# tdj28/ml-depth-pro-video

Hardware: AMD Instinct MI355X
Metric: frames/sec at 1536x1536 (1/2/4/8 MI355X) + depth L1 vs reference (higher is better)
Workload: dtype bf16+f16; 1 GPU; BASELINE config 2/3: one 1536x1536 frame per GPU per step through DepthPro.infer (patch+image+FOV ViT-L, decoder, heads), hipGraph replay; global_batch=1, parallelism=frame-dp1, graph=True

## Files before the change

ml-depth-pro-video_amd/csrc/dp_gemm.hip:

```cpp
#include "dp_gemm_impl.h"
#include "dp_ln_merge.h"

namespace dpg {
std::atomic<int> g_dbg_flags{0};

constexpr int DP_MAX_DEV = 64;
std::atomic<int> g_num_cu[DP_MAX_DEV];
int num_cus() {
  int dev = 0;
  if (hipGetDevice(&dev) != hipSuccess || dev < 0) dev = 0;
  std::atomic<int>& slot = g_num_cu[dev < DP_MAX_DEV ? dev : 0];
  int n = slot.load(std::memory_order_relaxed);
  if (n <= 0) {
    if (hipDeviceGetAttribute(&n, hipDeviceAttributeMultiprocessorCount, dev) != hipSuccess || n <= 0) n = 256;
    if (dev < DP_MAX_DEV) slot.store(n, std::memory_order_relaxed);
  }
  return n;
}
}

namespace {
int launch_tile(const GemmP& p, int tile, bool conv, bool bf16, void* ws, hipStream_t s) {
  switch (tile_info(tile).fam) {
    case FAM_SMALL: return launch_part_small(p, tile, conv, bf16, s);
    case FAM_BIG320: return launch_part_big320(p, tile, conv, bf16, s);
    case FAM_8PH: return launch_part_8ph(p, tile, conv, bf16, s);
    case FAM_8PH320: return launch_part_8ph320(p, conv, bf16, s);
    case FAM_PBIG: return launch_part_pbig(p, tile, conv, bf16, s);
    case FAM_SK: return launch_part_sk(p, conv, ws, bf16, s);
    case FAM_SPLITK: return launch_part_splitk(p, conv, bf16, s);
    case FAM_CV3: return launch_part_cv3(p, conv, bf16, s, tile_info(tile).bm / 16);
    default: return launch_part_big(p, tile, conv, bf16, s);
  }
}
}

extern "C" int dp_gemm_debug_flags(int flags) {
  g_dbg_flags.store(flags, std::memory_order_relaxed);
  return 0;
}

extern "C" int64_t dp_gemm_workspace_size(void) { return SK_FLAG_BYTES + (int64_t)SK_MAX_WG * SK_TILE_F * 4; }

namespace {
__global__ void __launch_bounds__(256) ln_merge_kernel(const float* __restrict__ part, int M, float eps,
                                                       float* __restrict__ out) {
  const int m = blockIdx.x * 256 + threadIdx.x;
  if (m >= M) return;
  const f32x4_t* pp = (const f32x4_t*)(part + (long long)m * 16);
  f32x4_t c[4];
  #pragma unroll
  for (int i = 0; i < 4; ++i) c[i] = pp[i];
  *(float2*)(out + 2LL * m) = ln_merge_row(c, eps);
}

__global__ void ws_check_kernel(uint32_t* __restrict__ ws, int32_t* __restrict__ status) {
  const uint32_t err = ws[DP_GEMM_WS_ERROR_OFFSET / 4];
  if (threadIdx.x == 0) status[0] = (int32_t)err;
  if (err == 0) return;
  __syncthreads();
  for (int i = threadIdx.x; i < (int)(SK_FLAG_BYTES / 4); i += blockDim.x) ws[i] = 0u;
}
}

extern "C" int dp_gemm_workspace_check(void* workspace, int32_t* status, dp_stream_t stream) {
  if (!workspace || !status) return DP_ERR_ARG;
  hipLaunchKernelGGL(ws_check_kernel, dim3(1), dim3(256), 0, (hipStream_t)stream, (uint32_t*)workspace, status);
  DP_CHECK_LAUNCH();
  return 0;
}

namespace {
struct PlanFacts {
  bool conv, k3s1p1, sq3x3, hps, hps4, bc, lnp, lnc, ws_ok, col8_shape, col8_align, off32, dcv;
  long long tiles256;
  unsigned c_bytes, dcv_bytes;
};

PlanFacts plan_facts(const dp_gemm_args* a) {
  PlanFacts f{};
  f.conv = a->a_mode == DP_A_CONV;
  f.k3s1p1 = f.conv && a->k_h == 3 && a->k_w == 3 && a->stride == 1 && a->pad == 1;
  f.sq3x3 = f.k3s1p1 && a->in_h == a->in_w && a->out_h == a->in_h && a->out_w == a->in_w && a->in_w % 16 == 0 &&
            a->in_c % 64 == 0 && (long long)a->M * a->in_c < (1LL << 30);
  f.hps = a->store_mode == DP_STORE_HEAD_PS;
  f.hps4 = f.k3s1p1 && f.hps && a->K == 4 * a->in_c;
  f.bc = a->store_mode == DP_STORE_ROWS && a->head_corr;
  f.lnp = a->ln_part_out || a->ln_xb_out || a->ln_xl || a->ln_rs_out;
  f.lnc = a->ln_part_in || a->ln_colsum || a->ln_rs_in;
  f.ws_ok = a->workspace && a->workspace_bytes >= dp_gemm_workspace_size();
  f.col8_shape = a->N % 8 == 0 && !(a->store_mode == DP_STORE_DECONV2X2 && a->dc_cout % 8 != 0);
  f.col8_align = !(a->c_dtype != DP_F32 && a->ldc % 8 != 0) && !(a->R1 && a->ldr1 % 8 != 0) &&
                 !(a->R2 && a->ldr2 % 8 != 0);
  f.tiles256 = (long long)((a->M + 255) / 256) * (a->N / 256);
  if (a->store_mode == DP_STORE_ROWS && !a->head_w && !a->head_corr) {
    long long last = a->M - 1;
    if (a->row_group) last = (last / a->row_group) * a->row_group_out + a->row_off + last % a->row_group;
    const long long ext = (last * a->ldc + a->N) * (a->c_dtype == DP_F32 ? 4 : 2);
    if (ext < 0xFFFFFF00LL) f.c_bytes = (unsigned)ext;
  }
  if (a->store_mode == DP_STORE_DECONV2X2 && a->c_dtype != DP_F32) {
    const long long ext = ((4LL * a->M - 1) * a->ldc + a->dc_cout) * 2;
    if (ext < 0xFFFFFF00LL) f.dcv_bytes = (unsigned)ext;
  }
  f.off32 = (a->a_mode != DP_A_DENSE || (long long)a->M * a->lda < (1LL << 31)) &&
            (long long)a->N * a->ldb < (1LL << 31);
  if (!f.off32) f.c_bytes = f.dcv_bytes = 0;
  f.dcv = a->store_mode == DP_STORE_DECONV2X2 && !a->relu_a && !a->gamma && a->act == DP_ACT_NONE &&
          a->dc_w >= 8;
  return f;
}

int validate(const dp_gemm_args* a, const PlanFacts& f) {
  if (a->M <= 0 || a->N <= 0 || a->K <= 0) return DP_ERR_SHAPE;
  if (a->K % BK != 0 || a->N % 4 != 0) return DP_ERR_SHAPE;
  if (a->ldb % 8 != 0 || (a->a_mode == DP_A_DENSE && a->lda % 8 != 0)) return DP_ERR_ALIGN;
  if ((!a->head_w && !f.hps && a->ldc % 4 != 0) || (a->R1 && a->ldr1 % 4 != 0) ||
      (a->R2 && a->ldr2 % 4 != 0) || (a->pos && a->ldpos % 4 != 0))
    return DP_ERR_ALIGN;
  if (!a->A || !a->B || (!a->C && !a->ln_xl)) return DP_ERR_ARG;
  if (a->dtype != DP_BF16 && a->dtype != DP_F16) return DP_ERR_DTYPE;
  if (a->c_dtype != DP_BF16 && a->c_dtype != DP_F16 && a->c_dtype != DP_F32) return DP_ERR_DTYPE;
  if (a->c_dtype != DP_F32 && a->c_dtype != a->dtype) return DP_ERR_DTYPE;
  if (a->accumulate && a->c_dtype != DP_F32) return DP_ERR_DTYPE;
  if (a->pos && (a->pos_group <= 0)) return DP_ERR_ARG;
  if (f.conv) {
    if (a->in_c % BK != 0 || (a->k_h * a->k_w * a->in_c != a->K && !f.hps4)) return DP_ERR_SHAPE;
    if (a->out_h <= 0 || a->out_w <= 0 || a->stride <= 0 || a->M % (a->out_h * a->out_w) != 0)
      return DP_ERR_SHAPE;
  }
  if (f.hps) {
    if (!f.conv || a->N != 128 || !a->head_w || !a->head_corr || a->c_dtype != DP_F32 ||
        a->accumulate || a->R1 || a->R2 || a->pos || a->gamma || a->act != DP_ACT_NONE)
      return DP_ERR_ARG;
  }
  if (f.bc) {
    if (!f.k3s1p1 || a->head_w || a->relu_a ||
        a->row_group || a->out_h != a->in_h || a->out_w != a->in_w || a->N % 8 != 0 || a->N < 128 ||
        (a->tile != DP_TILE_AUTO && a->tile <= DP_TILE_256x32))
      return DP_ERR_ARG;
  }
  if (a->store_mode == DP_STORE_DECONV2X2) {
    if (a->dc_cout % 4 != 0 || a->N != 4 * a->dc_cout || a->dc_h <= 0 || a->dc_w <= 0 ||
        a->M % (a->dc_h * a->dc_w) != 0)
      return DP_ERR_SHAPE;
  }
  if (f.lnp && f.lnc) return DP_ERR_ARG;
  if (f.lnp && !a->ln_xl && (!a->ln_part_out || !a->ln_xb_out || !a->accumulate || !a->C || a->c_dtype != DP_F32 ||
                             a->act != DP_ACT_NONE || a->N % 256 != 0))
    return DP_ERR_ARG;
  if (a->ln_xl && (!a->ln_xb_out || !a->accumulate || a->c_dtype != DP_F32 || a->act != DP_ACT_NONE ||
                   a->N % 256 != 0 || a->ldc % 8 != 0 || (long long)a->M * a->ldc * 4 >= 0xFFFFFF00LL))
    return DP_ERR_ARG;
  if (f.lnc && (!(a->ln_part_in || a->ln_rs_in) || (a->ln_part_in && a->ln_rs_in) || !a->ln_colsum || a->K != 1024 ||
                a->accumulate || a->c_dtype == DP_F32 || a->gamma || (a->act != DP_ACT_NONE && a->act != DP_ACT_GELU) ||
                !(a->ln_eps > 0.f)))
    return DP_ERR_ARG;
  if (a->ln_rs_out && (!a->ln_xl || !a->ln_part_out || a->N != 1024 || !(a->ln_eps > 0.f) || !f.ws_ok ||
                       (a->M + 319) / 320 > 1023 - LN_CNT_WORD))
    return DP_ERR_ARG;
  if (a->ln_rs_in && a->tile != DP_TILE_AUTO && a->tile != DP_TILE_P8PH_256x256) return DP_ERR_ARG;
  if ((f.lnp || f.lnc) && a->tile != DP_TILE_AUTO && a->tile != DP_TILE_8PH_320x256 &&
      !(f.lnc && a->tile == DP_TILE_P8PH_256x256))
    return DP_ERR_ARG;
  return 0;
}

int col8_rc(const PlanFacts& f, int tile) {
  if (tile < 0 || !tile_info(tile).col8) return 0;
  return !f.col8_shape ? DP_ERR_SHAPE : !f.col8_align ? DP_ERR_ALIGN : 0;
}
bool serves_streamk(const dp_gemm_args* a, const PlanFacts& f) { return f.ws_ok && a->N % 256 == 0; }
bool serves_splitk(const dp_gemm_args* a, const PlanFacts& f, int& split) {
  if (!f.ws_ok || a->N % 256 != 0 || a->store_mode != DP_STORE_ROWS || a->row_group || a->head_w || a->head_corr ||
      f.lnp || f.lnc) return false;
  const long long slab = (long long)a->M * a->N * 4, slabs = (a->workspace_bytes - SK_FLAG_BYTES) / slab;
  split = (int)std::min({num_cus() / f.tiles256, (long long)(a->K / BK / 2), slabs, 32LL});
  return true;
}

bool serves_pbig(const dp_gemm_args* a, const PlanFacts& f) { return f.c_bytes && a->N % 256 == 0; }

bool serves_p8ph(const dp_gemm_args* a, const PlanFacts& f, int dbg) {
  return a->a_mode == DP_A_DENSE && a->N % 256 == 0 && a->K >= 128 && a->c_dtype != DP_F32 &&
         ((a->store_mode == DP_STORE_ROWS && f.c_bytes) || (f.dcv && f.dcv_bytes)) && !a->R1 && !a->R2 && !a->pos &&
         !a->accumulate && !a->row_group && !a->head_w && !a->head_corr && !(dbg & DBG_NO_FAST_EPILOGUE);
}

bool serves_8ph320(const dp_gemm_args* a, const PlanFacts& f, int dbg) {
  const bool plain = a->a_mode == DP_A_DENSE && !a->relu_a && a->N % 256 == 0 && a->store_mode == DP_STORE_ROWS &&
                     !a->R1 && !a->R2 && !a->pos && !a->row_group && !a->head_w && !a->head_corr &&
                     !(dbg & DBG_NO_FAST_EPILOGUE) && f.off32;
  const bool epi_ok = (!a->accumulate && a->c_dtype != DP_F32) ||
                      (a->accumulate && a->c_dtype == DP_F32 && a->act == DP_ACT_NONE);
  return plain && epi_ok;
}

bool cv3_shape(const dp_gemm_args* a, const PlanFacts& f, int th) {
  if (!f.sq3x3 || a->out_w % th != 0 || a->row_group || (a->head_w && !f.hps) || a->gamma || a->pos || a->accumulate)
    return false;
  if (!f.hps && a->store_mode != DP_STORE_ROWS) return false;
  if (f.hps4 && a->relu_a) return false;
  if (f.bc && (a->c_dtype == DP_F32 || a->R1 || a->R2 || a->N % 128 != 0)) return false;
  if (!f.hps && !f.bc && (a->c_dtype == DP_F32 || a->N % 256 != 0)) return false;
  return th == 12 ? !(f.hps || f.bc) : th == 24 ? (f.hps || f.bc) && a->N == 128 : true;
}
bool serves_cv3(const dp_gemm_args* a, const PlanFacts& f, int th) {
  return cv3_shape(a, f, th) && (a->act == DP_ACT_NONE || a->act == DP_ACT_RELU) && (long long)a->N * a->ldb < (1LL << 31);
}

int choose_auto(const dp_gemm_args* a, const PlanFacts& f, int dbg) {
  auto ncu = [n = 0LL]() mutable { return n ? n : n = num_cus(); };
  const long long tiles256 = f.tiles256, tiles320 = (long long)((a->M + 319) / 320) * (a->N / 256);
  int tile;
  if (a->N <= 32) tile = DP_TILE_256x32;
  else if (a->N <= 64) tile = DP_TILE_256x64;
  else if (!f.col8_shape || !f.col8_align) tile = DP_TILE_128x128;
  else if (a->N == 128 && a->M >= 512 * 256) {
    tile = !f.bc || (dbg & DBG_NO_CV3_HEAD) ? DP_TILE_BIG_512x128 : cv3_shape(a, f, 24) ? DP_TILE_CV3_384x128
           : cv3_shape(a, f, 16) ? DP_TILE_CV3_256x256 : DP_TILE_BIG_512x128;
  }
  else if (a->N % 256 != 0) tile = DP_TILE_BIG_256x128;
  else if (serves_streamk(a, f) && f.conv && !(dbg & DBG_NO_SMALL_STREAMK) && tiles256 < ncu() && a->K >= 4608) {
    tile = DP_TILE_STREAMK_256x256;
  } else if (serves_streamk(a, f) && a->K <= 256 && tiles256 >= 1024) {
    tile = DP_TILE_STREAMK_256x256;
  } else {
    const long long tiles128 = (long long)((a->M + 255) / 256) * (a->N / 128);
    const long long cost256 = (tiles256 + ncu() - 1) / ncu() * 256 * 20, cost320 = (tiles320 + ncu() - 1) / ncu() * 320 * 20;
    const long long cost128 = (tiles128 + ncu() - 1) / ncu() * 128 * 23;
    if (cost128 < cost256 && cost128 < cost320) tile = DP_TILE_BIG_256x128;
    else if (cost320 < cost256) tile = DP_TILE_BIG_320x256;
    else tile = (tiles256 >= 600 && !f.conv) ? DP_TILE_8PH_256x256 : DP_TILE_BIG_256x256;
    if (tile == DP_TILE_8PH_256x256 && (dbg & DBG_FC1_BIG320)) tile = DP_TILE_BIG_320x256;
    else if (tile == DP_TILE_8PH_256x256 && (dbg & DBG_FC1_BIG256)) tile = DP_TILE_BIG_256x256;
  }
  if (serves_pbig(a, f) && !(dbg & DBG_NO_PBIG)) {
    const bool dense_ok = f.conv || (dbg & DBG_PBIG_DENSE);
    if (dense_ok && tile == DP_TILE_BIG_320x256 && tiles320 >= 2 * ncu()) tile = DP_TILE_PBIG_320x256;
    else if (dense_ok && tile == DP_TILE_BIG_256x256 && tiles256 >= 2 * ncu()) tile = DP_TILE_PBIG_256x256;
  }
  if (f.dcv && f.col8_shape && f.col8_align && !(dbg & DBG_NO_P8PH_DECONV) && tiles256 >= 128) tile = DP_TILE_P8PH_256x256;
  else if (tile == DP_TILE_8PH_256x256 && !(dbg & DBG_NO_P8PH) && serves_p8ph(a, f, dbg)) tile = DP_TILE_P8PH_256x256;
  if (tile == DP_TILE_BIG_320x256 && !(dbg & DBG_NO_8PH320) && serves_8ph320(a, f, dbg)) tile = DP_TILE_8PH_320x256;
  if (!(dbg & DBG_NO_CV3) && !f.bc && a->N % 256 == 0 && f.col8_align && cv3_shape(a, f, 16) && f.off32 &&
      a->act != DP_ACT_GELU) {
    const long long t16 = (long long)(a->M / 256) * (a->N / 256);
    if (t16 >= 4 * ncu()) tile = DP_TILE_CV3_256x256;
    else if (cv3_shape(a, f, 12)) {
      const long long t12 = (long long)(a->M / ((long long)a->in_w * a->in_w)) * (a->in_w / 12) * (a->in_w / 16) * (a->N / 256);
      if (t12 >= 2 * ncu() && t12 % ncu() == 0 && t16 % ncu() != 0) tile = DP_TILE_CV3_192x256;
      else if (t12 <= ncu() && 2 * t12 >= ncu()) tile = DP_TILE_CV3_192x256;
    }
  }
  return tile;
}

void fill_params(const dp_gemm_args* a, const PlanFacts& f, int tile, int ksplit, int dbg, GemmP& p) {
  p.M = a->M; p.N = a->N; p.K = a->K;
  p.A = (const u16*)a->A; p.lda = a->lda;
  p.B = (const u16*)a->B; p.ldb = a->ldb;
  p.relu_a = a->relu_a;
  p.in_h = a->in_h; p.in_w = a->in_w; p.in_c = a->in_c; p.k_h = a->k_h; p.k_w = a->k_w;
  p.stride = a->stride; p.pad = a->pad; p.out_h = a->out_h; p.out_w = a->out_w;
  p.bias = a->bias; p.act = a->act; p.gamma = a->gamma;
  p.pos = a->pos; p.ldpos = a->ldpos; p.pos_group = a->pos_group; p.pos_off = a->pos_off;
  p.R1 = (const u16*)a->R1; p.ldr1 = a->ldr1; p.R2 = (const u16*)a->R2; p.ldr2 = a->ldr2;
  p.C = a->C; p.ldc = a->ldc; p.c_dtype = a->c_dtype; p.accumulate = a->accumulate;
  p.store_mode = a->store_mode; p.dc_h = a->dc_h; p.dc_w = a->dc_w; p.dc_cout = a->dc_cout;
  p.row_group = a->row_group; p.row_group_out = a->row_group_out; p.row_off = a->row_off;
  p.head_w = a->head_w; p.head_b = a->head_b; p.head_corr = a->head_corr;
  p.ln_part_out = a->ln_part_out; p.ln_xb_out = (u16*)a->ln_xb_out; p.ln_xl = (u16*)a->ln_xl;
  p.ln_part_in = a->ln_part_in; p.ln_colsum = a->ln_colsum; p.ln_eps = a->ln_eps;
  p.ln_rs = a->ln_rs_in; p.ln_rs_out = a->ln_rs_out;
  p.ln_cnt = a->ln_rs_out ? (unsigned*)a->workspace + LN_CNT_WORD : nullptr;
  p.tiles_n = p.tiles_m = 1;
  if (tile == DP_TILE_STREAMK_256x256) p.tiles_n = a->N / 256, p.tiles_m = (a->M + 255) / 256;
  p.dbg = dbg;
  p.c_bytes = tile == DP_TILE_P8PH_256x256 && f.dcv ? f.dcv_bytes : f.c_bytes;
  p.ksplit = ksplit;
  p.kpart = ksplit > 1 ? (float*)((char*)a->workspace + SK_FLAG_BYTES) : nullptr;
  p.groups = 1;
}

int gemm_plan(const dp_gemm_args* a, GemmP& p, int& tile) {
  if (!a) return DP_ERR_ARG;
  const PlanFacts f = plan_facts(a);
  if (const int rc = validate(a, f)) return rc;
  const int dbg = g_dbg_flags.load(std::memory_order_relaxed);
  tile = a->tile;
  if (a->ln_rs_in) tile = DP_TILE_P8PH_256x256;
  if (f.hps) {
    if (f.hps4) {
      if (tile == DP_TILE_AUTO) tile = a->out_w % 48 == 0 ? DP_TILE_CV3_384x128 : DP_TILE_CV3_256x256;
      else if (tile != DP_TILE_CV3_256x256 && tile != DP_TILE_CV3_384x128) return DP_ERR_ARG;
    } else if (tile != DP_TILE_CV3_256x256 && tile != DP_TILE_CV3_384x128 && tile != DP_TILE_BIG_256x128)
      tile = a->M >= 512 * 256 ? DP_TILE_BIG_512x128 : DP_TILE_BIG_256x128;
  } else if (a->head_w) {
    if (a->N > 32 || a->store_mode != DP_STORE_ROWS) return DP_ERR_SHAPE;
    tile = DP_TILE_256x32;
  }
  if (const int rc = col8_rc(f, tile)) return rc;
  if (tile == DP_TILE_AUTO) tile = choose_auto(a, f, dbg);
  int ksplit = 1;
  switch (tile) {
    case DP_TILE_STREAMK_256x256: if (!serves_streamk(a, f)) return DP_ERR_ARG; break;
    case DP_TILE_SPLITK_256x256: if (!serves_splitk(a, f, ksplit)) return DP_ERR_ARG;
      if (ksplit < 2) return DP_ERR_SHAPE;
      break;
    case DP_TILE_PBIG_320x256: case DP_TILE_PBIG_256x256: if (!serves_pbig(a, f)) return DP_ERR_ARG; break;
    case DP_TILE_P8PH_256x256: if (!serves_p8ph(a, f, dbg)) return DP_ERR_ARG; break;
  }
  const bool lnc_p8 = f.lnc && tile == DP_TILE_P8PH_256x256 && (f.ws_ok || a->ln_rs_in) && !(dbg & DBG_LNC_8PH320) &&
                      (a->ln_rs_in || (long long)(a->M + 255) / 256 * 256 * 8 <= (long long)SK_TILE_F * 4);
  if (a->ln_rs_in && !lnc_p8) return DP_ERR_ARG;
  if ((f.lnp || f.lnc) && !lnc_p8) tile = DP_TILE_8PH_320x256;
  if (tile == DP_TILE_8PH_320x256 && !serves_8ph320(a, f, dbg)) return DP_ERR_ARG;
  if (const int rc = col8_rc(f, tile)) return rc;
  if (tile_info(tile).fam == FAM_CV3 && !serves_cv3(a, f, tile_info(tile).bm / 16)) return DP_ERR_ARG;
  if (f.bc && tile != DP_TILE_BIG_512x128 && tile != DP_TILE_CV3_256x256 && tile != DP_TILE_CV3_384x128) return DP_ERR_ARG;
  fill_params(a, f, tile, ksplit, dbg, p);
  return 0;
}
}

extern "C" int dp_gemm_plan(const dp_gemm_args* a, int32_t* tile_out, int32_t* grid_out) {
  GemmP p;
  int tile = 0;
  if (const int rc = gemm_plan(a, p, tile)) return rc;
  const TileInfo& t = tile_info(tile);
  int grid = ((a->M + t.bm - 1) / t.bm) * ((a->N + t.bn - 1) / t.bn);
  if (t.cu_capped) grid = std::min(grid, num_cus());
  if (t.fam == FAM_SPLITK) grid *= p.ksplit;
  if (t.fam == FAM_SK) grid = sk_grid(p);
  if (tile_out) *tile_out = tile;
  if (grid_out) *grid_out = grid;
  return 0;
}

extern "C" int dp_gemm(const dp_gemm_args* a, dp_stream_t stream) {
  GemmP p;
  int tile = 0;
  if (const int rc = gemm_plan(a, p, tile)) return rc;
  hipStream_t s = (hipStream_t)stream;
  const bool conv = a->a_mode == DP_A_CONV;
  if (tile == DP_TILE_P8PH_256x256 && a->ln_part_in && !a->ln_rs_in) {
    float* rs = (float*)((char*)a->workspace + SK_FLAG_BYTES);
    hipLaunchKernelGGL(ln_merge_kernel, dim3((a->M + 255) / 256), dim3(256), 0, s, a->ln_part_in, a->M, a->ln_eps, rs);
    DP_CHECK_LAUNCH();
    p.ln_rs = rs;
  }
  return launch_tile(p, tile, conv, a->dtype == DP_BF16, a->workspace, s);
}

extern "C" int dp_gemm_grouped(const dp_gemm_args* a, int32_t groups, dp_stream_t stream) {
  if (!a || groups < 1 || groups > DP_MAX_GROUPS) return DP_ERR_ARG;
  if (groups == 1) return dp_gemm(a, stream);
  GemmP p;
  for (int g = 0; g < groups; ++g) {
    GemmP q;
    int t = 0;
    const int rc = gemm_plan(&a[g], q, t);
    if (rc) return rc;
    const dp_gemm_args &x = a[0], &y = a[g];
    if (y.M != x.M || y.N != x.N || y.K != x.K || y.dtype != x.dtype || y.lda != x.lda || y.ldb != x.ldb ||
        y.a_mode != DP_A_DENSE || x.a_mode != DP_A_DENSE || y.relu_a || y.act != x.act ||
        !y.bias != !x.bias || !y.gamma != !x.gamma || !y.pos != !x.pos || y.ldpos != x.ldpos ||
        y.pos_group != x.pos_group || y.pos_off != x.pos_off || !y.R1 != !x.R1 || y.ldr1 != x.ldr1 ||
        !y.R2 != !x.R2 || y.ldr2 != x.ldr2 || y.ldc != x.ldc || y.c_dtype != x.c_dtype ||
        y.accumulate != x.accumulate || y.store_mode != DP_STORE_ROWS || x.store_mode != DP_STORE_ROWS ||
        y.row_group != x.row_group || y.row_group_out != x.row_group_out || y.row_off != x.row_off ||
        y.head_w || y.head_corr || y.N % 8 != 0 || y.ln_part_out || y.ln_xb_out || y.ln_xl || y.ln_part_in ||
        y.ln_rs_out || y.ln_rs_in ||
        y.ln_colsum)
      return DP_ERR_ARG;
    if (g == 0) p = q;
    p.grp[g] = GemmP::Group{q.A, q.B, q.bias, q.gamma, q.pos, q.R1, q.R2, q.C};
  }
  p.groups = groups;
  hipStream_t s = (hipStream_t)stream;
  return launch_part_big(p, TILE_GRP_128x128, false, a->dtype == DP_BF16, s);
}
```

ml-depth-pro-video_amd/csrc/dp_gemm_big.h:

```cpp
#pragma once

#include "dp_gemm_dev.h"
#include "dp_gemm_epilogue.h"

namespace {

template <typename K_, int BM, int BN, int BKT, int NS, bool PIPE, bool CONV, bool RELU, int NW = 8, int EACT = -1,
          bool GRP = false, bool SPLIT = false>
__global__ void __launch_bounds__(NW * 64, NW == 4 ? 2 : 1) gemm_big_kernel(const GemmP p_arg) {
  constexpr int WN = NW == 4 ? 2 : (BM == 512 ? 2 : 4), WM = NW / WN;
  constexpr int TM = BM / WM, TN = BN / WN;
  constexpr int FM = TM / 16, FN = TN / 16;
  constexpr int RB = BKT * 2;
  constexpr int CR = BKT / 8;
  constexpr int ROWS_PER_WAVE_PIECE = 1024 / RB;
  constexpr int ROWS_PER_ROUND = NW * ROWS_PER_WAVE_PIECE;
  constexpr int A_BYTES = BM * RB, B_BYTES = BN * RB;
  constexpr int STAGE = A_BYTES + B_BYTES;
  constexpr int LA = BM / ROWS_PER_ROUND;
  constexpr int LB = BN / ROWS_PER_ROUND;
  constexpr int LT = LA + LB;
  constexpr int EPI_BYTES = NW * 32 * (TN + 4) * 4;
  constexpr int SMEM = NS * STAGE > EPI_BYTES ? NS * STAGE : EPI_BYTES;
  static_assert(NS >= 2 && SMEM <= 160 * 1024 && LB >= 1, "LDS ring");
  __shared__ __attribute__((aligned(1024))) char smem[SMEM];

  const int tid = threadIdx.x, lane = tid & 63;
  const int wave = tid >> 6;
  const int wave_u = __builtin_amdgcn_readfirstlane(wave);
  const int wm = wave / WN, wn = wave % WN;

  const int nwg = gridDim.x, bid = blockIdx.x;
  const int xcd = bid & 7, q8 = nwg >> 3, r8 = nwg & 7;
  int wgid = (xcd < r8 ? xcd * (q8 + 1) : r8 * (q8 + 1) + (xcd - r8) * q8) + (bid >> 3);
  GemmP p_grp;
  if constexpr (GRP) {
    const int per = p_arg.tiles_m * p_arg.tiles_n;
    const int g = wgid / per;
    wgid -= g * per;
    p_grp = p_arg;
    const GemmP::Group& q = p_arg.grp[g];
    p_grp.A = q.A; p_grp.B = q.B; p_grp.bias = q.bias; p_grp.gamma = q.gamma; p_grp.pos = q.pos;
    p_grp.R1 = q.R1; p_grp.R2 = q.R2; p_grp.C = q.C;
  }
  int kbeg = 0, kcnt = p_arg.K / BKT;
  if constexpr (SPLIT) {
    const int per = p_arg.tiles_m * p_arg.tiles_n;
    const int sp = wgid / per;
    wgid -= sp * per;
    const int kt_all = p_arg.K / BKT;
    kbeg = sp * kt_all / p_arg.ksplit;
    kcnt = (sp + 1) * kt_all / p_arg.ksplit - kbeg;
    p_grp = p_arg;
    p_grp.C = p_arg.kpart + (long long)sp * p_arg.M * p_arg.N;
    p_grp.ldc = p_arg.N; p_grp.c_dtype = DP_F32; p_grp.accumulate = 0; p_grp.store_mode = DP_STORE_ROWS;
    p_grp.bias = nullptr; p_grp.gamma = nullptr; p_grp.pos = nullptr; p_grp.R1 = nullptr; p_grp.R2 = nullptr;
    p_grp.act = DP_ACT_NONE; p_grp.row_group = 0; p_grp.head_w = nullptr; p_grp.head_corr = nullptr;
  }
  const GemmP& p = (GRP || SPLIT) ? p_grp : p_arg;
  int tile_m, tile_n;
  tile_coords(p, wgid, tile_m, tile_n);
  const int m0 = tile_m * BM, n0 = tile_n * BN;
  DP_STAMPS_DECL;
  DP_STAMP(st0_);

  const int prow = wave * ROWS_PER_WAVE_PIECE + lane / CR;
  const int pchunk = BKT == 64 ? ((lane & 7) ^ ((lane >> 3) & 7)) : ((lane & 3) ^ ((lane >> 3) & 3));
  const u16* a_src[LA];
  ConvRow a_cr[LA];
  #pragma unroll
  for (int i = 0; i < LA; ++i) {
    const int m = m0 + i * ROWS_PER_ROUND + prow;
    if constexpr (CONV) {
      a_cr[i] = conv_row(p, m);
    } else {
      a_src[i] = p.A + (long long)(m < p.M ? m : p.M - 1) * p.lda + pchunk * 8;
    }
  }
  const u16* b_src[LB];
  #pragma unroll
  for (int i = 0; i < LB; ++i) {
    const int n = n0 + i * ROWS_PER_ROUND + prow;
    b_src[i] = p.B + (long long)(n < p.N ? n : p.N - 1) * p.ldb + pchunk * 8;
  }
  const uint32_t lds_base = __builtin_amdgcn_readfirstlane(lds_addr(smem)) + wave_u * 1024;
  auto issue = [&](int kt, int stage) {
    const uint32_t sa = lds_base + stage * STAGE;
    const uint32_t sb = sa + A_BYTES;
    const int k0 = (kt + kbeg) * BKT;
    int t_ky = 0, t_kx = 0, t_ci = 0;
    if constexpr (CONV) conv_tap(p, k0, t_ky, t_kx, t_ci);
    #pragma unroll
    for (int i = 0; i < LA; ++i) {
      const void* src;
      if constexpr (CONV) {
        bool inb;
        const u16* s = conv_src(p, a_cr[i], t_ky, t_kx, t_ci + pchunk * 8, inb);
        src = inb ? (const void*)s : (const void*)g_zero_page;
      } else {
        src = a_src[i] + k0;
      }
      glds16(src, sa + i * NW * 1024);
    }
    #pragma unroll
    for (int i = 0; i < LB; ++i) glds16(b_src[i] + k0, sb + i * NW * 1024);
  };

  f32x4_t acc[FM][FN];
  #pragma unroll
  for (int i = 0; i < FM; ++i)
    #pragma unroll
    for (int j = 0; j < FN; ++j) acc[i][j] = f32x4_t{0.f, 0.f, 0.f, 0.f};

  const int frow = lane & 15, fchunk = lane >> 4;
  constexpr int KS = BKT / 32;
  auto compute = [&](int stage) {
    const u16* sa = (const u16*)(smem + stage * STAGE);
    const u16* sb = (const u16*)(smem + stage * STAGE + A_BYTES);
    #pragma unroll
    for (int ks = 0; ks < KS; ++ks) {
      uint4 bf[FN];
      #pragma unroll
      for (int j = 0; j < FN; ++j)
        bf[j] = *(const uint4*)(sb + lds_off_t<BKT>(wn * TN + j * 16 + frow, ks * 4 + fchunk));
      uint4 afs[FM];
      #pragma unroll
      for (int i = 0; i < FM; ++i) afs[i] = *(const uint4*)(sa + lds_off_t<BKT>(wm * TM + i * 16 + frow, ks * 4 + fchunk));
      __builtin_amdgcn_s_setprio(1);
      #pragma unroll
      for (int i = 0; i < FM; ++i) {
        uint4 af = afs[i];
        if constexpr (RELU) af = relu_pk16(af);
        #pragma unroll
        for (int j = 0; j < FN; ++j) acc[i][j] = K_::mfma16(bf[j], af, acc[i][j]);
      }
      __builtin_amdgcn_s_setprio(0);
    }
  };

  const int KT = kcnt;
  auto nxt = [&](int st) { return st + 1 == NS ? 0 : st + 1; };
  auto wait_tile = [&](int t) { wait_vmcnt_le<(NS - 2) * LT>(min(NS - 2, KT - 1 - t) * LT); };
  if constexpr (!PIPE) {
    #pragma unroll
    for (int t = 0; t < NS - 1; ++t)
      if (t < KT) issue(t, t);
    int stage = 0;
    for (int kt = 0; kt < KT; ++kt) {
      wait_tile(kt);
      lds_barrier();
#ifdef DP_STAMPS
      if (kt == 0) DP_STAMP(st1_);
#endif
      if (kt + NS - 1 < KT && !(p.dbg & DBG_NO_LOOP_LOADS)) {
        const int st = stage + NS - 1;
        issue(kt + NS - 1, st >= NS ? st - NS : st);
      }
      if (p.dbg & DBG_NO_MFMA) {
        const u16* sa = (const u16*)(smem + stage * STAGE);
        uint4 t = *(const uint4*)(sa + lds_off_t<BKT>(wm * TM + frow, fchunk));
        asm volatile("" ::"v"(t.x));
      } else {
        compute(stage);
      }
      stage = nxt(stage);
    }
  } else {
    uint4 fa0[FM], fb0[FN], fa1[FM], fb1[FN];
    auto rd = [&](uint4 (&fa)[FM], uint4 (&fb)[FN], int stg, int ks) {
      const u16* sa = (const u16*)(smem + stg * STAGE);
      const u16* sb = (const u16*)(smem + stg * STAGE + A_BYTES);
      #pragma unroll
      for (int j = 0; j < FN; ++j)
        fb[j] = *(const uint4*)(sb + lds_off_t<BKT>(wn * TN + j * 16 + frow, ks * 4 + fchunk));
      #pragma unroll
      for (int i = 0; i < FM; ++i)
        fa[i] = *(const uint4*)(sa + lds_off_t<BKT>(wm * TM + i * 16 + frow, ks * 4 + fchunk));
    };
    auto mma = [&](const uint4 (&fa)[FM], const uint4 (&fb)[FN]) {
      __builtin_amdgcn_s_setprio(1);
      #pragma unroll
      for (int i = 0; i < FM; ++i) {
        uint4 a = fa[i];
        if constexpr (RELU) a = relu_pk16(a);
        #pragma unroll
        for (int j = 0; j < FN; ++j) acc[i][j] = K_::mfma16(fb[j], a, acc[i][j]);
      }
      __builtin_amdgcn_s_setprio(0);
    };
    #pragma unroll
    for (int t = 0; t < NS - 1; ++t)
      if (t < KT) issue(t, t);
    wait_tile(0);
    lds_barrier();
    DP_STAMP(st1_);
    rd(fa0, fb0, 0, 0);
    int stage = 0;
    if constexpr (KS == 2) {
      for (int kt = 0; kt < KT; ++kt) {
        if (kt + NS - 1 < KT) {
          int st = stage + NS - 1;
          issue(kt + NS - 1, st >= NS ? st - NS : st);
        }
        rd(fa1, fb1, stage, 1);
        mma(fa0, fb0);
        const int nst = nxt(stage);
        if (kt + 1 < KT) {
          wait_tile(kt + 1);
          lds_barrier();
          rd(fa0, fb0, nst, 0);
        }
        mma(fa1, fb1);
        stage = nst;
      }
    } else {
      for (int kt = 0; kt < KT; kt += 2) {
        if (kt + NS - 1 < KT) {
          int st = stage + NS - 1;
          issue(kt + NS - 1, st >= NS ? st - NS : st);
        }
        int nst = nxt(stage);
        if (kt + 1 < KT) {
          wait_tile(kt + 1);
          lds_barrier();
          rd(fa1, fb1, nst, 0);
        }
        mma(fa0, fb0);
        stage = nst;
        if (kt + 1 >= KT) break;
        if (kt + NS < KT) {
          int st = stage + NS - 1;
          issue(kt + NS, st >= NS ? st - NS : st);
        }
        nst = nxt(stage);
        if (kt + 2 < KT) {
          wait_tile(kt + 2);
          lds_barrier();
          rd(fa0, fb0, nst, 0);
        }
        mma(fa1, fb1);
        stage = nst;
      }
    }
  }

  DP_STAMP(st2_);
  if (p.dbg & DBG_NO_EPILOGUE) {
    #pragma unroll
    for (int i = 0; i < FM; ++i)
      #pragma unroll
      for (int j = 0; j < FN; ++j) asm volatile("" ::"v"(acc[i][j][0]), "v"(acc[i][j][1]), "v"(acc[i][j][2]), "v"(acc[i][j][3]));
    return;
  }
  if constexpr (EACT >= EPI_ACC) {
    epilogue_acc32<EACT - EPI_ACC, FM, FN>(p, acc, lane, m0 + wm * TM, n0 + wn * TN);
    return;
  } else if constexpr (EACT >= 0) {
    lds_barrier();
    constexpr int PF = (FM * 16 * TN * 2 * NW <= SMEM) ? FM : FM / 2;
    epilogue_mfma<K_, EACT, FM, FN, TN, PF>(p, acc, smem + wave * (PF * 16 * TN * 2), lane, m0 + wm * TM,
                                            n0 + wn * TN);
    return;
  }
  lds_barrier();
  constexpr int SROW = TN + 4;
  constexpr int CPR = TN / 8;
  constexpr int RPI = 64 / CPR;
  float* stg = (float*)smem + wave * (32 * SROW);
  constexpr int NIT = 32 / RPI;
  const int c8 = (lane % CPR) * 8, n_l = n0 + wn * TN + c8;
  ColConst cc;
  load_colconst(p, n_l, cc);
  #pragma unroll
  for (int q = 0; q < FM / 2; ++q) {
    #pragma unroll
    for (int i = 0; i < 2; ++i)
      #pragma unroll
      for (int j = 0; j < FN; ++j)
        *(f32x4_t*)(stg + (i * 16 + (lane & 15)) * SROW + j * 16 + 4 * (lane >> 4)) = acc[2 * q + i][j];
    constexpr int NITC = FM >= 8 && NIT > 2 ? 2 : NIT;
    #pragma unroll
    for (int c0 = 0; c0 < NIT; c0 += NITC) {
      float v[NITC][8];
      int ms[NITC];
      #pragma unroll
      for (int it = 0; it < NITC; ++it) {
        const int row = (c0 + it) * RPI + lane / CPR;
        const f32x4_t lo = *(const f32x4_t*)(stg + row * SROW + c8);
        const f32x4_t hi = *(const f32x4_t*)(stg + row * SROW + c8 + 4);
        #pragma unroll
        for (int r = 0; r < 4; ++r) { v[it][r] = lo[r]; v[it][4 + r] = hi[r]; }
        ms[it] = m0 + wm * TM + q * 32 + row;
      }
      if constexpr (TN % 32 == 0) {
        if (p.store_mode == DP_STORE_HEAD_PS) {
          head_ps_rows<NITC>(p, cc, ms, n_l, v, lane);
          continue;
        }
      }
      epilogue_rows<K_, NITC, CONV && BM == 512 && !RELU>(p, cc, ms, n_l, v);
    }
  }
  DP_STAMP(st3_);
  DP_STAMP_SAVE(wgid);
}

template <typename K_, int BM, int BN, int BKT, int NS, bool PIPE>
int launch_big(const GemmP& p0, bool conv, hipStream_t s) {
  GemmP p = p0;
  p.tiles_n = (p.N + BN - 1) / BN;
  p.tiles_m = (p.M + BM - 1) / BM;
  dim3 grid(p.tiles_n * p.tiles_m);
  int ea = BKT == 64 ? fast_epi_act(p) : -1;
  if (ea >= EPI_ACC && p.N % BN != 0) ea = -1;
  if (p.groups > 1) {
    if constexpr ((BM == 256 || BM == 128) && BN == 128 && BKT == 64 && NS == 3 && PIPE) {
      if (conv || p.relu_a) return DP_ERR_ARG;
      dim3 g(p.tiles_n * p.tiles_m * p.groups);
#define DP_GRP(E_) hipLaunchKernelGGL((gemm_big_kernel<K_, BM, BN, 64, 3, true, false, false, 8, E_, true>), g, dim3(NT_BIG), 0, s, p)
      if (ea == DP_ACT_NONE) DP_GRP(DP_ACT_NONE);
      else if (ea == DP_ACT_GELU) DP_GRP(DP_ACT_GELU);
      else if (ea == EPI_ACC) DP_GRP(EPI_ACC);
      else DP_GRP(-1);
#undef DP_GRP
      DP_CHECK_LAUNCH();
      return 0;
    } else {
      return DP_ERR_ARG;
    }
  }
#define DP_BIGE(C_, R_, E_) hipLaunchKernelGGL((gemm_big_kernel<K_, BM, BN, BKT, NS, PIPE, C_, R_, 8, E_>), grid, dim3(NT_BIG), 0, s, p)
#define DP_BIG(C_, R_) do { \
    if (ea < 0) DP_BIGE(C_, R_, -1); \
    else if constexpr (BKT == 64) { \
      if (ea == DP_ACT_NONE) DP_BIGE(C_, R_, DP_ACT_NONE); \
      else if (ea == DP_ACT_RELU) DP_BIGE(C_, R_, DP_ACT_RELU); \
      else if (ea == DP_ACT_GELU) DP_BIGE(C_, R_, DP_ACT_GELU); \
      else if constexpr (!C_ && !R_) { if (ea == EPI_ACC) DP_BIGE(C_, R_, EPI_ACC); else DP_BIGE(C_, R_, -1); } \
      else DP_BIGE(C_, R_, -1); } \
  } while (0)
  if (conv && p.relu_a) DP_BIG(true, true);
  else if (conv) DP_BIG(true, false);
  else if (p.relu_a) DP_BIG(false, true);
  else DP_BIG(false, false);
#undef DP_BIG
#undef DP_BIGE
  DP_CHECK_LAUNCH();
  return 0;
}

}
```

ml-depth-pro-video_amd/csrc/dp_gemm_epilogue.h:

```cpp
#pragma once

#include "dp_gemm_impl.h"

namespace {

__device__ __forceinline__ void add8_f32(float (&v)[8], const float* p) {
  const float4 a = *(const float4*)p, b = *(const float4*)(p + 4);
  v[0] += a.x; v[1] += a.y; v[2] += a.z; v[3] += a.w;
  v[4] += b.x; v[5] += b.y; v[6] += b.z; v[7] += b.w;
}

struct ColConst {
  float b[8], g[8];
};
__device__ __forceinline__ void load_colconst(const GemmP& p, int n, ColConst& c) {
  const bool ok = n < p.N;
  if (p.bias && ok) {
    const float4 x = *(const float4*)(p.bias + n), y = *(const float4*)(p.bias + n + 4);
    c.b[0] = x.x; c.b[1] = x.y; c.b[2] = x.z; c.b[3] = x.w; c.b[4] = y.x; c.b[5] = y.y; c.b[6] = y.z; c.b[7] = y.w;
  } else {
    #pragma unroll
    for (int r = 0; r < 8; ++r) c.b[r] = 0.f;
  }
  if (p.gamma && ok) {
    const float4 x = *(const float4*)(p.gamma + n), y = *(const float4*)(p.gamma + n + 4);
    c.g[0] = x.x; c.g[1] = x.y; c.g[2] = x.z; c.g[3] = x.w; c.g[4] = y.x; c.g[5] = y.y; c.g[6] = y.z; c.g[7] = y.w;
  } else {
    #pragma unroll
    for (int r = 0; r < 8; ++r) c.g[r] = 1.f;
  }
}
__device__ __forceinline__ long long out_offset(const GemmP& p, int m, int n) {
  if (p.store_mode == DP_STORE_DECONV2X2) {
    const int hw = p.dc_h * p.dc_w;
    const int b = m / hw, rr = m - b * hw;
    const int y = rr / p.dc_w, x = rr - y * p.dc_w;
    const int q = n / p.dc_cout, co = n - q * p.dc_cout;
    const long long pix = ((long long)b * 2 * p.dc_h + 2 * y + (q >> 1)) * (2 * p.dc_w) + 2 * x + (q & 1);
    return pix * p.ldc + co;
  }
  long long row = m;
  if (p.row_group) row = (long long)(m / p.row_group) * p.row_group_out + p.row_off + m % p.row_group;
  return row * p.ldc + n;
}
template <typename K_>
__device__ __forceinline__ void add8_u4(float (&v)[8], uint4 r) {
  const uint32_t w[4] = {r.x, r.y, r.z, r.w};
  #pragma unroll
  for (int k = 0; k < 4; ++k) {
    v[2 * k] += K_::to_f(w[k] & 0xffff);
    v[2 * k + 1] += K_::to_f(w[k] >> 16);
  }
}
__device__ __forceinline__ void border_correct(const GemmP& p, int m, int nc, float (&z)[8]) {
  const int hw = p.out_h * p.out_w;
  const int rr = m % hw;
  const int yy = rr / p.out_w, xx = rr - yy * p.out_w;
  const bool top = yy == 0, bot = yy == p.out_h - 1, lft = xx == 0, rgt = xx == p.out_w - 1;
  if (!(top || bot || lft || rgt)) return;
  #pragma unroll 1
  for (int t = 0; t < 9; ++t) {
    const int a = t / 3, c = t - 3 * (t / 3);
    const bool oob = (a == 0 && top) || (a == 2 && bot) || (c == 0 && lft) || (c == 2 && rgt);
    if (oob) {
      const float4 lo = *(const float4*)(p.head_corr + t * p.N + nc);
      const float4 hi = *(const float4*)(p.head_corr + t * p.N + nc + 4);
      z[0] -= lo.x; z[1] -= lo.y; z[2] -= lo.z; z[3] -= lo.w;
      z[4] -= hi.x; z[5] -= hi.y; z[6] -= hi.z; z[7] -= hi.w;
    }
  }
}
template <typename K_, int NIT, bool BC = false>
__device__ __forceinline__ void epilogue_rows(const GemmP& p, const ColConst& cc, const int (&ms)[NIT], int n,
                                              float (&v)[NIT][8]) {
  const int nc = n < p.N ? n : p.N - 8;
  int mc[NIT];
  long long off[NIT];
  #pragma unroll
  for (int it = 0; it < NIT; ++it) {
    mc[it] = ms[it] < p.M ? ms[it] : p.M - 1;
    off[it] = out_offset(p, mc[it], nc);
  }
  uint4 r1[NIT], r2[NIT];
  float4 c0[NIT], c1[NIT];
  if (p.R1) {
    #pragma unroll
    for (int it = 0; it < NIT; ++it) r1[it] = *(const uint4*)(p.R1 + (long long)mc[it] * p.ldr1 + nc);
  }
  if (p.R2) {
    #pragma unroll
    for (int it = 0; it < NIT; ++it) r2[it] = *(const uint4*)(p.R2 + (long long)mc[it] * p.ldr2 + nc);
  }
  const bool acc32 = p.accumulate && p.c_dtype == DP_F32;
  if (acc32) {
    #pragma unroll
    for (int it = 0; it < NIT; ++it) {
      const float* c = (const float*)p.C + off[it];
      c0[it] = *(const float4*)c;
      c1[it] = *(const float4*)(c + 4);
    }
  }
  #pragma unroll
  for (int it = 0; it < NIT; ++it) {
    float (&x)[8] = v[it];
    #pragma unroll
    for (int r = 0; r < 8; ++r) x[r] += cc.b[r];
    if constexpr (BC) {
      if (p.head_corr) border_correct(p, mc[it], nc, x);
    }
    if (p.act == DP_ACT_RELU) {
      #pragma unroll
      for (int r = 0; r < 8; ++r) x[r] = fmaxf(x[r], 0.f);
    } else if (p.act == DP_ACT_GELU) {
      #pragma unroll
      for (int r = 0; r < 8; ++r) x[r] = gelu_erf(x[r]);
    }
    if (p.gamma) {
      #pragma unroll
      for (int r = 0; r < 8; ++r) x[r] *= cc.g[r];
    }
    if (p.pos) add8_f32(x, p.pos + (long long)(mc[it] % p.pos_group + p.pos_off) * p.ldpos + nc);
    if (p.R1) add8_u4<K_>(x, r1[it]);
    if (p.R2) add8_u4<K_>(x, r2[it]);
    if (acc32) {
      x[0] += c0[it].x; x[1] += c0[it].y; x[2] += c0[it].z; x[3] += c0[it].w;
      x[4] += c1[it].x; x[5] += c1[it].y; x[6] += c1[it].z; x[7] += c1[it].w;
    }
  }
  const bool nok = n < p.N;
  #pragma unroll
  for (int it = 0; it < NIT; ++it) {
    const float (&x)[8] = v[it];
    if (!(nok && ms[it] < p.M)) continue;
    if (p.c_dtype == DP_F32) {
      float* c = (float*)p.C + off[it];
      *(float4*)c = make_float4(x[0], x[1], x[2], x[3]);
      *(float4*)(c + 4) = make_float4(x[4], x[5], x[6], x[7]);
    } else {
      uint4 o;
      o.x = (uint32_t)K_::from_f(x[0]) | ((uint32_t)K_::from_f(x[1]) << 16);
      o.y = (uint32_t)K_::from_f(x[2]) | ((uint32_t)K_::from_f(x[3]) << 16);
      o.z = (uint32_t)K_::from_f(x[4]) | ((uint32_t)K_::from_f(x[5]) << 16);
      o.w = (uint32_t)K_::from_f(x[6]) | ((uint32_t)K_::from_f(x[7]) << 16);
      *(uint4*)((u16*)p.C + off[it]) = o;
    }
  }
}

template <typename K_, int ACT, int FM, int FN, int TN, int PF>
__device__ __forceinline__ void epilogue_mfma(const GemmP& p, f32x4_t (&acc)[FM][FN], char* slab, int lane,
                                              int m_base, int n_base) {
  constexpr int CH = TN / 8;
  constexpr int RPI = 64 / CH;
  static_assert(FM % PF == 0 && (CH == 16 || CH == 8 || CH == 4), "tile");
  const int t = lane & 15, g = lane >> 4;
  float bias[FN][4], gam[FN][4];
  #pragma unroll
  for (int fn = 0; fn < FN; ++fn) {
    const int n = n_base + fn * 16 + 4 * g;
    const bool ok = n < p.N;
    const float4 b = (p.bias && ok) ? *(const float4*)(p.bias + n) : make_float4(0.f, 0.f, 0.f, 0.f);
    const float4 q = (p.gamma && ok) ? *(const float4*)(p.gamma + n) : make_float4(1.f, 1.f, 1.f, 1.f);
    bias[fn][0] = b.x; bias[fn][1] = b.y; bias[fn][2] = b.z; bias[fn][3] = b.w;
    gam[fn][0] = q.x; gam[fn][1] = q.y; gam[fn][2] = q.z; gam[fn][3] = q.w;
  }
  #pragma unroll
  for (int f0 = 0; f0 < FM; f0 += PF) {
    #pragma unroll
    for (int fm = 0; fm < PF; ++fm)
      #pragma unroll
      for (int fn = 0; fn < FN; ++fn) {
        f32x4_t x = acc[f0 + fm][fn] + f32x4_t{bias[fn][0], bias[fn][1], bias[fn][2], bias[fn][3]};
        if constexpr (ACT == DP_ACT_RELU) {
          #pragma unroll
          for (int r = 0; r < 4; ++r) x[r] = fmaxf(x[r], 0.f);
        } else if constexpr (ACT == DP_ACT_GELU) {
          x = gelu_erf4(x);
        }
        x = x * f32x4_t{gam[fn][0], gam[fn][1], gam[fn][2], gam[fn][3]};
        const int row = fm * 16 + t;
        const int chunk = fn * 2 + (g >> 1);
        uint2 w;
        w.x = K_::pack2(x[0], x[1]);
        w.y = K_::pack2(x[2], x[3]);
        *(uint2*)(slab + row * (TN * 2) + ((chunk ^ (row & (CH - 1))) << 4) + (g & 1) * 8) = w;
      }
    #pragma unroll
    for (int k = 0; k < PF * 16 / RPI; ++k) {
      const int row = k * RPI + lane / CH, chunk = lane % CH;
      const uint4 d = *(const uint4*)(slab + row * (TN * 2) + ((chunk ^ (row & (CH - 1))) << 4));
      const int m = m_base + f0 * 16 + row, n = n_base + chunk * 8;
      if (m < p.M && n < p.N) *(uint4*)((u16*)p.C + (long long)m * p.ldc + n) = d;
    }
  }
}

template <int ACT, int FM, int FN>
__device__ __forceinline__ void epilogue_acc32(const GemmP& p, f32x4_t (&acc)[FM][FN], int lane, int m_base,
                                               int n_base) {
  #pragma clang fp contract(off)
  const int t = lane & 15, g = lane >> 4;
  float bias[FN][4], gam[FN][4];
  #pragma unroll
  for (int fn = 0; fn < FN; ++fn) {
    const int n = n_base + fn * 16 + 4 * g;
    const bool ok = n < p.N;
    const float4 b = (p.bias && ok) ? *(const float4*)(p.bias + n) : make_float4(0.f, 0.f, 0.f, 0.f);
    const float4 q = (p.gamma && ok) ? *(const float4*)(p.gamma + n) : make_float4(1.f, 1.f, 1.f, 1.f);
    bias[fn][0] = b.x; bias[fn][1] = b.y; bias[fn][2] = b.z; bias[fn][3] = b.w;
    gam[fn][0] = q.x; gam[fn][1] = q.y; gam[fn][2] = q.z; gam[fn][3] = q.w;
  }
  float* const C = (float*)p.C;
  f32x4_t cur[FN], nxt[FN];
  auto load_row = [&](int fm, f32x4_t (&c)[FN]) __attribute__((always_inline)) {
    const int m = min(m_base + fm * 16 + t, p.M - 1);
    #pragma unroll
    for (int fn = 0; fn < FN; ++fn) c[fn] = *(const f32x4_t*)(C + (long long)m * p.ldc + n_base + fn * 16 + 4 * g);
  };
  load_row(0, cur);
  #pragma unroll
  for (int fm = 0; fm < FM; ++fm) {
    if (fm + 1 < FM) load_row(fm + 1, nxt);
    const int m = m_base + fm * 16 + t;
    #pragma unroll
    for (int fn = 0; fn < FN; ++fn) {
      f32x4_t x;
      #pragma unroll
      for (int r = 0; r < 4; ++r) {
        float v = acc[fm][fn][r] + bias[fn][r];
        if constexpr (ACT == DP_ACT_RELU) v = fmaxf(v, 0.f);
        else if constexpr (ACT == DP_ACT_GELU) v = gelu_erf(v);
        x[r] = v * gam[fn][r] + cur[fn][r];
      }
      if (m < p.M) *(f32x4_t*)(C + (long long)m * p.ldc + n_base + fn * 16 + 4 * g) = x;
    }
    #pragma unroll
    for (int fn = 0; fn < FN; ++fn) cur[fn] = nxt[fn];
  }
}

template <int NIT>
__device__ __forceinline__ void head_ps_rows(const GemmP& p, const ColConst& cc, const int (&ms)[NIT], int n,
                                             float (&v)[NIT][8], int lane) {
  const int q = n >> 5, o0 = n & 31, dy = q >> 1, dx = q & 1;
  const int hw = p.out_h * p.out_w;
  float hw8[8];
  #pragma unroll
  for (int r = 0; r < 8; ++r) hw8[r] = p.head_w[o0 + r];
  #pragma unroll
  for (int it = 0; it < NIT; ++it) {
    const int m = ms[it] < p.M ? ms[it] : p.M - 1;
    const int b = m / hw, rr = m - b * hw;
    const int y = rr / p.out_w, x = rr - y * p.out_w;
    float z[8];
    #pragma unroll
    for (int r = 0; r < 8; ++r) z[r] = v[it][r] + cc.b[r];
    const bool top = y == 0 && dy == 0, bot = y == p.out_h - 1 && dy == 1;
    const bool lft = x == 0 && dx == 0, rgt = x == p.out_w - 1 && dx == 1;
    if (top || bot || lft || rgt) {
      #pragma unroll
      for (int a = 0; a < 3; ++a)
        #pragma unroll
        for (int c = 0; c < 3; ++c) {
          const bool oob = (a == 0 && top) || (a == 2 && bot) || (c == 0 && lft) || (c == 2 && rgt);
          if (oob) {
            #pragma unroll
            for (int r = 0; r < 8; ++r) z[r] -= p.head_corr[(a * 3 + c) * 32 + o0 + r];
          }
        }
    }
    float hs = 0.f;
    #pragma unroll
    for (int r = 0; r < 8; ++r) hs += fmaxf(z[r], 0.f) * hw8[r];
    hs += __shfl_xor(hs, 1);
    hs += __shfl_xor(hs, 2);
    if ((lane & 3) == 0 && ms[it] < p.M) {
      const long long W2 = 2LL * p.out_w;
      ((float*)p.C)[((long long)b * 2 * p.out_h + 2 * y + dy) * W2 + 2 * x + dx] = fmaxf(hs + p.head_b, 0.f);
    }
  }
}

}
```

ml-depth-pro-video_amd/csrc/dp_gemm_impl.h:

```cpp
#pragma once

#include "dp_common.h"

#include <atomic>

namespace dpg {

constexpr int BK = 64;
typedef unsigned int u32x4_t __attribute__((ext_vector_type(4)));
typedef unsigned int u32x2_t __attribute__((ext_vector_type(2)));

constexpr int DP_MAX_GROUPS = 4;

struct GemmP {
  int M, N, K;
  const u16* A;
  long long lda;
  const u16* B;
  long long ldb;
  int relu_a;
  int in_h, in_w, in_c, k_h, k_w, stride, pad, out_h, out_w;
  const float* bias;
  int act;
  const float* gamma;
  const float* pos;
  long long ldpos;
  int pos_group, pos_off;
  const u16* R1;
  long long ldr1;
  const u16* R2;
  long long ldr2;
  void* C;
  long long ldc;
  int c_dtype;
  int accumulate;
  int store_mode;
  int dc_h, dc_w, dc_cout;
  int row_group, row_group_out, row_off;
  const float* head_w;
  float head_b;
  const float* head_corr;
  int tiles_n, tiles_m;
  int dbg;
  unsigned c_bytes;
  float* ln_part_out;
  u16* ln_xb_out;
  u16* ln_xl;
  const float* ln_part_in;
  const float* ln_colsum;
  float ln_eps;
  const float* ln_rs;
  float* ln_rs_out;
  unsigned* ln_cnt;
  int groups;
  int ksplit;
  float* kpart;
  struct Group {
    const u16* A;
    const u16* B;
    const float* bias;
    const float* gamma;
    const float* pos;
    const u16* R1;
    const u16* R2;
    void* C;
  } grp[DP_MAX_GROUPS];
};

extern std::atomic<int> g_dbg_flags;
enum : int {
  DBG_NO_EPILOGUE = 1,
  DBG_NO_LOOP_LOADS = 2,
  DBG_NO_MFMA = 4,
  DBG_ROW_MAJOR_TILES = 16,
  DBG_NO_SMALL_STREAMK = 32,
  DBG_SK_GIVE_UP = 64,
  DBG_NO_PBIG = 1024,
  DBG_PBIG_DENSE = 2048,
  DBG_NO_CV3_HEAD = 4096,
  DBG_FC1_BIG320 = 8192,
  DBG_FC1_BIG256 = 16384,
  DBG_NO_8PH320 = 1 << 15,
  DBG_NO_CV3 = 1 << 16,
  DBG_BAND8 = 1 << 18,
  DBG_BAND2 = 1 << 19,
  DBG_NO_FAST_EPILOGUE = 1 << 20,
  DBG_NO_P8PH = 1 << 22,
  DBG_NO_P8PH_DECONV = 1 << 23,
  DBG_CV3_ABLATION = 1 << 24,
  DBG_LNC_8PH320 = 1 << 25,
  DBG_HILO_AHEAD1 = 1 << 27,
};
constexpr int DBG_CV3_ABLATION_MASK = 2047;
int num_cus();

enum TileFamily { FAM_NONE, FAM_SMALL, FAM_BIG, FAM_BIG320, FAM_8PH, FAM_8PH320, FAM_PBIG, FAM_SK, FAM_SPLITK, FAM_CV3 };
struct TileInfo {
  int bm, bn;
  TileFamily fam;
  bool cu_capped, col8;
};
constexpr TileInfo TILES[] = {
    {0, 0, FAM_NONE, false, false},
    {128, 128, FAM_SMALL, false, false},
    {256, 64, FAM_SMALL, false, false},
    {256, 32, FAM_SMALL, false, false},
    {256, 256, FAM_BIG, false, true},
    {256, 128, FAM_BIG, false, true},
    {256, 256, FAM_BIG, false, true},
    {256, 128, FAM_BIG, false, true},
    {256, 256, FAM_8PH, false, true},
    {256, 256, FAM_BIG, false, true},
    {256, 256, FAM_BIG, false, true},
    {256, 128, FAM_BIG, false, true},
    {256, 256, FAM_SK, false, true},
    {320, 256, FAM_BIG320, false, true},
    {512, 128, FAM_BIG320, false, true},
    {320, 256, FAM_PBIG, true, true},
    {256, 256, FAM_PBIG, true, true},
    {256, 128, FAM_SMALL, false, true},
    {256, 256, FAM_8PH, true, true},
    {320, 256, FAM_8PH320, false, true},
    {256, 256, FAM_CV3, false, true},
    {256, 256, FAM_SPLITK, false, true},
    {192, 256, FAM_CV3, false, true},
    {384, 128, FAM_CV3, false, true},
};
constexpr int N_TILES = sizeof(TILES) / sizeof(TILES[0]);
static_assert(N_TILES == 24 && DP_TILE_CV3_384x128 == N_TILES - 1, "one entry per DP_TILE_*");
inline const TileInfo& tile_info(int tile) { return TILES[tile >= 0 && tile < N_TILES ? tile : DP_TILE_BIG_256x256]; }

int launch_part_big(const GemmP& p, int tile, bool conv, bool bf16, hipStream_t s);
constexpr int TILE_GRP_128x128 = -1;
int launch_part_big320(const GemmP& p, int tile, bool conv, bool bf16, hipStream_t s);
int launch_part_8ph(const GemmP& p, int tile, bool conv, bool bf16, hipStream_t s);
int launch_part_8ph320(const GemmP& p, bool conv, bool bf16, hipStream_t s);
int launch_part_cv3(const GemmP& p, bool conv, bool bf16, hipStream_t s, int th = 16);
int launch_part_pbig(const GemmP& p, int tile, bool conv, bool bf16, hipStream_t s);
int launch_part_small(const GemmP& p, int tile, bool conv, bool bf16, hipStream_t s);
int launch_part_sk(const GemmP& p, bool conv, void* ws, bool bf16, hipStream_t s);
int launch_part_splitk(const GemmP& p, bool conv, bool bf16, hipStream_t s);
}

namespace {
using namespace dpg;

constexpr int SK_MIN_STEPS = 8, SK_MAX_SPLIT = 6;
int sk_grid(const GemmP& p) {
  const int tiles = p.tiles_m * p.tiles_n;
  int g = num_cus();
  if (g > 256) g = 256;
  if (tiles >= g) return g;
  if (p.dbg & DBG_NO_SMALL_STREAMK) return tiles;
  const int kt = p.K / 64;
  int s = g / tiles;
  if (s < 2) return kt >= 2 * SK_MIN_STEPS ? g : tiles;
  if (s > SK_MAX_SPLIT) s = SK_MAX_SPLIT;
  if (s > kt / SK_MIN_STEPS) s = kt / SK_MIN_STEPS;
  return tiles * (s < 1 ? 1 : s);
}

constexpr int SK_TILE_F = 256 * 256;
constexpr long long SK_FLAG_BYTES = 4096;
constexpr int LN_CNT_WORD = 512;
static_assert(DP_GEMM_WS_ERROR_OFFSET == 4 * 1023, "error word offset (dp_mi355x.h)");
constexpr int SK_MAX_WG = 256;

__host__ __device__ inline bool needs_rowld(const GemmP& p) {
  return p.R1 || p.R2 || p.pos || p.accumulate || p.store_mode != DP_STORE_ROWS || p.row_group || p.head_corr ||
         p.head_w;
}

constexpr int EPI_ACC = 16;
__host__ inline int fast_epi_act(const GemmP& p) {
  if (p.dbg & DBG_NO_FAST_EPILOGUE) return -1;
  if (!needs_rowld(p)) return p.c_dtype == DP_F32 ? -1 : p.act;
  const bool acc_only = p.accumulate && p.c_dtype == DP_F32 && !p.R1 && !p.R2 && !p.pos &&
                        p.store_mode == DP_STORE_ROWS && !p.row_group && !p.head_corr && !p.head_w;
  return acc_only ? EPI_ACC + p.act : -1;
}

}
```

ml-depth-pro-video_amd/csrc/dp_ln_merge.h:

```cpp
#pragma once

#include "dp_common.h"

namespace {

__device__ __forceinline__ float2 ln_merge_row(const f32x4_t (&c)[4], float eps) {
  const float mean = (((c[0][0] + c[0][2]) + (c[1][0] + c[1][2])) + ((c[2][0] + c[2][2]) + (c[3][0] + c[3][2]))) *
                     (1.f / 8);
  float m2 = 0.f;
  #pragma unroll
  for (int i = 0; i < 4; ++i) {
    const float d0 = c[i][0] - mean, d1 = c[i][2] - mean;
    m2 += (c[i][1] + 128.f * d0 * d0) + (c[i][3] + 128.f * d1 * d1);
  }
  const float rs = rsqrtf(m2 * (1.f / 1024) + eps);
  return make_float2(rs, -rs * mean);
}

}
```

ml-depth-pro-video_amd/depth_pro/engine.py:

```python

from __future__ import annotations

import os
from typing import Dict, Optional, Tuple

import torch

from . import ops
from ._lib import (DP_ACT_GELU, DP_ACT_RELU, DP_BF16, DP_F16, DP_F32, DP_TILE_P8PH_256x256, DP_TILE_SPLITK_256x256,
                   DPError, load)
from .spec import DEPTH, EMBED_DIM, HEADS, IMG_SIZE, MLP_DIM, TOKENS

_ABLATE = set(filter(None, os.environ.get("DP_ABLATE", "").split(",")))


def ln_fold_enabled() -> bool:
    return not ({"ln", "vitgemm"} & _ABLATE)


NWIN = 35
TOK = TOKENS
PTOK = TOKENS - 1
D = EMBED_DIM


def _conv_w(w: torch.Tensor, dt) -> torch.Tensor:
    return ops.conv_weight(w, dt)


def _deconv_w(w: torch.Tensor, dt) -> torch.Tensor:
    ci, co = w.shape[0], w.shape[1]
    return w.permute(2, 3, 1, 0).reshape(4 * co, ci).to(dt).contiguous()


def _f32(t: torch.Tensor) -> torch.Tensor:
    return t.detach().to(torch.float32).contiguous()


def compose_head(wd: torch.Tensor, bd: torch.Tensor, w2: torch.Tensor, b2: torch.Tensor, dt) -> Dict[str, object]:
    ci_n, c_n = wd.shape[0], wd.shape[1]
    o_n = w2.shape[0]
    wc = torch.zeros(4, o_n, 3, 3, ci_n, dtype=torch.float32, device=wd.device)
    for dy in range(2):
        for dx in range(2):
            q = 2 * dy + dx
            for a in range(-1, 2):
                ry = dy + a
                ty, py = ry // 2 + 1, ry & 1
                for b in range(-1, 2):
                    rx = dx + b
                    tx, px = rx // 2 + 1, rx & 1
                    wc[q, :, ty, tx, :] += w2[:, :, a + 1, b + 1] @ wd[:, :, py, px].t()
    corr = torch.einsum("ocab,c->abo", w2, bd).contiguous()
    bias = (b2 + corr.sum(dim=(0, 1))).repeat(4).contiguous()
    w_conv = wc.reshape(4 * o_n, 3, 3, ci_n).permute(0, 3, 1, 2)
    return {"head.ps.w": ops.conv_weight(w_conv, dt), "head.ps.w4": compact_head_w(wc, dt), "head.ps.b": bias,
            "head.ps.corr": corr.reshape(-1).contiguous()}


def compact_head_w(wc: torch.Tensor, dt) -> torch.Tensor:
    q_n, o_n, _, _, ci_n = wc.shape
    out = torch.empty(q_n, o_n, 4, ci_n, dtype=torch.float32, device=wc.device)
    for q in range(q_n):
        dy, dx = q >> 1, q & 1
        keep = torch.zeros(3, 3, dtype=torch.bool, device=wc.device)
        keep[dy:dy + 2, dx:dx + 2] = True
        if wc[q][:, ~keep].ne(0).any():
            raise AssertionError(f"composed head conv: parity {q} has a non-zero weight outside its 2 x 2 taps")
        out[q] = wc[q][:, dy:dy + 2, dx:dx + 2].reshape(o_n, 4, ci_n)
    return out.reshape(q_n * o_n, 4 * ci_n).to(dt).contiguous()


def compose_head0(w0: torch.Tensor, b0: torch.Tensor, wo: torch.Tensor, bo: torch.Tensor, dt) -> Dict[str, object]:
    wc = torch.einsum("omyx,mc->ocyx", w0, wo)
    corr = torch.einsum("omyx,m->yxo", w0, bo).contiguous()
    bias = (b0 + corr.sum(dim=(0, 1))).contiguous()
    return {"head.0c.w": ops.conv_weight(wc, dt), "head.0c.b": bias, "head.0c.corr": corr.reshape(-1).contiguous()}


def precision_codes(codes) -> Tuple[int, int]:
    if isinstance(codes, (tuple, list)):
        v, d = int(codes[0]), int(codes[1])
    else:
        v = d = int(codes)
    for c in (v, d):
        if c not in (DP_BF16, DP_F16):
            raise DPError("compute dtype must be bf16 or f16")
    return v, d


def pack_weights(sd: Dict[str, torch.Tensor], device: torch.device, dtype_code) -> Dict[str, object]:
    vcode, dcode = precision_codes(dtype_code)
    vdt, dt = ops.torch_dtype(vcode), ops.torch_dtype(dcode)
    g = lambda k: sd[k].detach().to(device)
    P: Dict[str, object] = {}
    fold = ln_fold_enabled()
    for vit in ("encoder.patch_encoder.", "encoder.image_encoder.", "fov.encoder.0."):
        if vit + "cls_token" not in sd:
            continue
        folded = fold and vit == "encoder.patch_encoder."
        P[vit + "cls"] = _f32(g(vit + "cls_token")).reshape(D)
        P[vit + "pos"] = _f32(g(vit + "pos_embed")).reshape(TOK, D)
        P[vit + "pe.w"] = g(vit + "patch_embed.proj.weight").reshape(D, -1).to(vdt).contiguous()
        P[vit + "pe.b"] = _f32(g(vit + "patch_embed.proj.bias"))
        for i in range(DEPTH):
            b = f"{vit}blocks.{i}."
            for n in ("norm1.weight", "norm1.bias", "norm2.weight", "norm2.bias", "attn.qkv.bias",
                      "attn.proj.bias", "mlp.fc1.bias", "mlp.fc2.bias", "ls1.gamma", "ls2.gamma"):
                P[b + n] = _f32(g(b + n))
            for n in ("attn.qkv.weight", "attn.proj.weight", "mlp.fc1.weight", "mlp.fc2.weight"):
                if folded and n in ("attn.qkv.weight", "mlp.fc1.weight"):
                    continue
                P[b + n] = g(b + n).to(vdt).contiguous()
        P[vit + "norm.weight"] = _f32(g(vit + "norm.weight"))
        P[vit + "norm.bias"] = _f32(g(vit + "norm.bias"))
        if folded:
            qg = ops.log2q_gamma(HEADS, D // HEADS, device)
            for i in range(DEPTH):
                b = f"{vit}blocks.{i}."
                for lin, ln, cs in (("attn.qkv", "norm1", qg), ("mlp.fc1", "norm2", None)):
                    wf, bf, sf = ops.fold_layernorm(g(b + lin + ".weight").float(), g(b + lin + ".bias").float(),
                                                    g(b + ln + ".weight").float(), g(b + ln + ".bias").float(),
                                                    vdt, cs)
                    P[b + lin + ".fold.w"], P[b + lin + ".fold.b"], P[b + lin + ".fold.s"] = wf, bf, sf
    for name, n_up in (("upsample_latent0", 3), ("upsample_latent1", 2), ("upsample0", 1),
                       ("upsample1", 1), ("upsample2", 1)):
        p = f"encoder.{name}."
        P[p + "0"] = _conv_w(g(p + "0.weight"), dt)
        for i in range(1, n_up + 1):
            P[p + str(i)] = _deconv_w(g(p + f"{i}.weight"), dt)
    P["encoder.upsample_lowres.w"] = _deconv_w(g("encoder.upsample_lowres.weight"), dt)
    P["encoder.upsample_lowres.b"] = _f32(g("encoder.upsample_lowres.bias")).repeat(4)
    P["encoder.fuse_lowres.w"] = _conv_w(g("encoder.fuse_lowres.weight"), dt)
    P["encoder.fuse_lowres.b"] = _f32(g("encoder.fuse_lowres.bias"))
    for i in range(1, 5):
        P[f"decoder.convs.{i}"] = _conv_w(g(f"decoder.convs.{i}.weight"), dt)
    for i in range(5):
        p = f"decoder.fusions.{i}."
        for r in ("resnet1", "resnet2"):
            for j in (1, 3):
                P[p + f"{r}.{j}.w"] = _conv_w(g(p + f"{r}.residual.{j}.weight"), dt)
                P[p + f"{r}.{j}.b"] = _f32(g(p + f"{r}.residual.{j}.bias"))
        wo = _f32(g(p + "out_conv.weight"))[:, :, 0, 0]
        bo = _f32(g(p + "out_conv.bias"))
        if i != 0:
            wd = _f32(g(p + "deconv.weight"))
            wc = torch.einsum("icyx,oc->ioyx", wd, wo)
            P[p + "up.w"] = _deconv_w(wc, dt)
            P[p + "up.b"] = bo.repeat(4)
        else:
            P[p + "out.w"] = wo.to(dt).contiguous()
            P[p + "out.b"] = bo
    P["head.0.w"] = _conv_w(g("head.0.weight"), dt)
    P["head.0.b"] = _f32(g("head.0.bias"))
    P.update(compose_head0(_f32(g("head.0.weight")), _f32(g("head.0.bias")),
                           _f32(g("decoder.fusions.0.out_conv.weight"))[:, :, 0, 0],
                           _f32(g("decoder.fusions.0.out_conv.bias")), dt))
    P.update(compose_head(_f32(g("head.1.weight")), _f32(g("head.1.bias")), _f32(g("head.2.weight")),
                          _f32(g("head.2.bias")), dt))
    P["head.4.w"] = _f32(g("head.4.weight")).reshape(-1)
    P["head.4.b"] = float(sd["head.4.bias"].detach().float().reshape(-1)[0])
    if "fov.encoder.1.weight" in sd:
        P["fov.lin.w"] = g("fov.encoder.1.weight").to(dt).contiguous()
        P["fov.lin.b"] = _f32(g("fov.encoder.1.bias"))
        P["fov.down.w"] = _conv_w(g("fov.downsample.0.weight"), dt)
        P["fov.down.b"] = _f32(g("fov.downsample.0.bias"))
        P["fov.h0.w"] = _conv_w(g("fov.head.0.weight"), dt)
        P["fov.h0.b"] = _f32(g("fov.head.0.bias"))
        P["fov.h2.w"] = _conv_w(g("fov.head.2.weight"), dt)
        P["fov.h2.b"] = _f32(g("fov.head.2.bias"))
        P["fov.h4.w"] = _f32(g("fov.head.4.weight")).reshape(-1)
        P["fov.h4.b"] = float(sd["fov.head.4.bias"].detach().float().reshape(-1)[0])
    return P


class _ViTBuffers:
    def __init__(self, rows: int, dt, dev, out_dt=None, ln_fold: bool = False):
        self.rows = rows
        self.x = torch.empty(rows, D, dtype=torch.float32, device=dev)
        self.part = torch.empty(rows, D // 128, 2, dtype=torch.float32, device=dev) if ln_fold else None
        self.h = torch.empty(rows, D, dtype=dt, device=dev)
        self.xl = torch.empty(rows, D, dtype=torch.int8, device=dev) if ln_fold else None
        self.rs = (torch.empty((rows + 255) // 256 * 256, 2, dtype=torch.float32, device=dev)
                   if ln_fold else None)
        self.qkv = torch.empty(rows, 3 * D, dtype=dt, device=dev)
        self.a = torch.empty(rows, D, dtype=dt, device=dev)
        self.m = torch.empty(rows, MLP_DIM, dtype=dt, device=dev)
        out_dt = out_dt or dt
        self.out = self.h if out_dt == dt else self.a.view(out_dt)


class _ViTRows:

    def __init__(self, buf: _ViTBuffers, lo: int, hi: int):
        self.rows = hi - lo
        self.x = buf.x[lo:hi]
        self.out = buf.out[lo:hi]


class FrameStatus:

    def __init__(self, frame: int, words: torch.Tensor, event: torch.cuda.Event):
        self.frame = frame
        self.words = words
        self.event = event
        self.reported = False
        self.owned = False

    def ready(self) -> bool:
        return self.event.query()

    def error(self) -> Optional[str]:
        self.event.synchronize()
        w = self.words.tolist()
        if any(w[:-1]):
            return ("dp_gemm: a stream-K partial-tile hand-off timed out in this forward "
                    "(workspace error word set): its depth map is invalid")
        if w[-1]:
            return f"{w[-1]} non-finite depth / focal-length value(s) in this frame's output"
        return None

    def check(self) -> None:
        msg = self.error()
        self.reported = True
        if msg is not None:
            raise DPError(f"frame {self.frame}: {msg}")

    def claim(self) -> "FrameStatus":
        self.owned = True
        return self


class BatchStatus:

    def __init__(self, frames: list):
        self.frames = list(frames)
        self.frame = self.frames[-1].frame if self.frames else -1

    @property
    def reported(self) -> bool:
        return all(f.reported for f in self.frames)

    def ready(self) -> bool:
        return all(f.ready() for f in self.frames)

    def claim(self) -> "BatchStatus":
        for f in self.frames:
            f.owned = True
        return self

    def error(self) -> Optional[str]:
        bad = [(f.frame, e) for f in self.frames for e in [f.error()] if e is not None]
        if not bad:
            return None
        return "; ".join(f"frame {n}: {e}" for n, e in bad)

    def check(self) -> None:
        msg = self.error()
        for f in self.frames:
            f.reported = True
        if msg is not None:
            raise DPError(msg)


class Engine:

    def __init__(self, packed: Dict[str, object], device: torch.device, dtype_code,
                 use_fov: bool = True):
        load()
        if device.type != "cuda":
            raise DPError("the MI355X Depth Pro engine needs a ROCm/HIP device")
        if device.index is None:
            device = torch.device("cuda", torch.cuda.current_device())
        self.vcode, self.code = precision_codes(dtype_code)
        if packed[next(k for k in packed if k.endswith("attn.qkv.weight"))].dtype != ops.torch_dtype(self.vcode) \
                or packed["decoder.convs.4"].dtype != ops.torch_dtype(self.code):
            raise DPError("packed weights were made for another compute precision")
        self.P = packed
        self.dev = device
        self.vdt = ops.torch_dtype(self.vcode)
        self.dt = ops.torch_dtype(self.code)
        self.use_fov = use_fov and "fov.lin.w" in packed
        dt, vdt, dev = self.dt, self.vdt, device
        e = lambda *s, dtype=None: torch.empty(*s, dtype=dtype or dt, device=dev)
        S = IMG_SIZE
        self.x0 = e(3, S, S, dtype=torch.float32)
        self.cols = e(NWIN * PTOK, 768, dtype=vdt)
        self.ln_fold = "encoder.patch_encoder.blocks.0.attn.qkv.fold.w" in packed
        if self.ln_fold != ln_fold_enabled():
            raise DPError("packed weights were made for the other LayerNorm path (DP_ABLATE differs from "
                          "when they were packed)")
        self.vp = _ViTBuffers(NWIN * TOK, vdt, dev, dt, ln_fold=self.ln_fold)
        self.side_vits = ["encoder.image_encoder."] + (["fov.encoder.0."] if self.use_fov else [])
        self.vs = _ViTBuffers(len(self.side_vits) * TOK, vdt, dev, dt)
        self.vi = _ViTRows(self.vs, 0, TOK)
        self.vf = _ViTRows(self.vs, TOK, 2 * TOK) if self.use_fov else None
        self.lat0 = e(96 * 96, D)
        self.lat1 = e(96 * 96, D)
        self.f0 = e(96 * 96, D)
        self.f1 = e(48 * 48, D)
        self.f2 = e(24 * 24, D)
        self.g = e(24 * 24, D)
        self.t96_256 = e(96 * 96, 256)
        self.t192_256 = e(192 * 192, 256)
        self.t384_256 = e(384 * 384, 256)
        self.enc0 = e(768 * 768, 256)
        self.t96_256b = e(96 * 96, 256)
        self.t192_256b = e(192 * 192, 256)
        self.enc1 = e(384 * 384, 256)
        self.t96_512 = e(96 * 96, 512)
        self.enc2 = e(192 * 192, 512)
        self.t48_1024 = e(48 * 48, D)
        self.enc3 = e(96 * 96, D)
        self.t24_1024 = e(24 * 24, D)
        self.cat = e(48 * 48, 2 * D)
        self.enc4 = e(48 * 48, D)
        self.dec = {}
        for s in (48, 96, 192, 384, 768):
            self.dec[s] = {k: e(s * s, 256) for k in ("c", "t", "x", "y")}
        self.low = self.dec[48]["c"]
        self.up = {s: e(s * s, 256) for s in (96, 192, 384, 768)}
        self.feats = e(768 * 768, 256)
        self.h0 = e(768 * 768, 128)
        self.canonical = e(1, 1, S, S, dtype=torch.float32)
        self.fov_tok = e(PTOK, 128)
        self.fx = e(24 * 24, 128)
        self.f12 = e(12 * 12, 64)
        self.f6 = e(6 * 6, 32)
        self.fov_deg = e(1, 1, 1, 1, dtype=torch.float32)
        self.graph: Optional[torch.cuda.CUDAGraph] = None
        self.side = torch.cuda.Stream(device=dev)
        self.dec_a = torch.cuda.Stream(device=dev)
        self.dec_b = torch.cuda.Stream(device=dev)
        self.dec_c = torch.cuda.Stream(device=dev)
        self.ws_main = ops.gemm_workspace(dev)
        self.ws_dec = ops.gemm_workspace(dev)
        self.head0_compose = os.environ.get("DP_HEAD0_COMPOSE", "1") == "1" and "head.0c.w" in packed
        self.head_ps_compact = os.environ.get("DP_HEAD_PS_COMPACT", "1") == "1" and "head.ps.w4" in packed
        self.qkv_gamma = ops.log2q_gamma(HEADS, D // HEADS, dev)
        self.serial_side = False
        self._wss = [self.ws_main, self.ws_dec]
        self.status_dev = torch.zeros(len(self._wss) + 1, dtype=torch.int32, device=dev)
        self._frames = 0
        self._recent: list = []
        self._unreported: list = []
        self.last_status: Optional[FrameStatus] = None
        self.sync_check = os.environ.get("DP_CHECK_SYNC", "0") == "1"
        self.qkv_tile = DP_TILE_P8PH_256x256

    def _vit(self, pres, buf: _ViTBuffers, n_img: int, cols_off_rows: int, hooks=None):
        for _ in self._vit_steps(pres, buf, n_img, cols_off_rows, hooks):
            pass

    def _vit_steps(self, pres, buf: _ViTBuffers, n_img: int, cols_off_rows: int, hooks=None):
        P, M = self.P, n_img * TOK
        G = len(pres)
        ln_on = "ln" not in _ABLATE and not (G > 1 and "sideln" in _ABLATE)
        gemm_on = "vitgemm" not in _ABLATE

        def lin(A, key, C, N, K, a_rows=True, **kw):
            per = {k: kw.pop(k) for k in ("bias", "gamma", "pos") if isinstance(kw.get(k), str)}
            A_off = kw.pop("A_off", 0)
            groups = []
            for g, pre in enumerate(pres):
                d = dict(A=A, B=P[pre + key], C=C, A_off=A_off + (g * M * K if a_rows else 0), C_off=g * M * N)
                d.update({k: P[pre + v] for k, v in per.items()})
                groups.append(d)
            ops.gemm_grouped(groups, M=kw.pop("M", M), N=N, K=K, **kw)

        def norm(key, out):
            ops.layernorm_grouped(buf.x, [P[pre + key + ".weight"] for pre in pres],
                                  [P[pre + key + ".bias"] for pre in pres], out, M, D)

        lin(self.cols, "pe.w", buf.x, D, 768, a_rows=False, M=n_img * PTOK, A_off=cols_off_rows * 768,
            bias="pe.b", pos="pos", ldpos=D, pos_group=PTOK, pos_off=1, row_group=PTOK, row_group_out=TOK,
            row_off=1)
        for g, pre in enumerate(pres):
            ops.vit_cls_rows(buf.x[g * M:], P[pre + "cls"], P[pre + "pos"], n_img)
        if G == 1 and buf.part is not None:
            yield from self._vit_blocks_folded(pres[0], buf, M, hooks)
            return
        yield
        for i in range(DEPTH):
            b = f"blocks.{i}."
            if ln_on:
                norm(b + "norm1", buf.h)
            if gemm_on:
                lin(buf.h, b + "attn.qkv.weight", buf.qkv, 3 * D, D, bias=b + "attn.qkv.bias", gamma=self.qkv_gamma)
            if "attn" not in _ABLATE:
                ops.attention(buf.qkv, buf.a, G * n_img, TOK, HEADS, D // HEADS, log2q=True)
            if gemm_on:
                lin(buf.a, b + "attn.proj.weight", buf.x, D, D, bias=b + "attn.proj.bias", gamma=b + "ls1.gamma",
                    accumulate=True)
            if ln_on:
                norm(b + "norm2", buf.h)
            if gemm_on:
                lin(buf.h, b + "mlp.fc1.weight", buf.m, MLP_DIM, D, bias=b + "mlp.fc1.bias", act=DP_ACT_GELU)
            if gemm_on:
                lin(buf.m, b + "mlp.fc2.weight", buf.x, D, MLP_DIM, bias=b + "mlp.fc2.bias", gamma=b + "ls2.gamma",
                    accumulate=True)
            if hooks and i in hooks:
                hooks[i]()
            if i == DEPTH - 1:
                norm("norm", buf.out)
            yield

    def _vit_blocks_folded(self, pre: str, buf: _ViTBuffers, M: int, hooks=None):
        P = self.P
        n_img = M // TOK
        ops.layernorm_stats(buf.x, buf.h, buf.part, M, D, xl=buf.xl)
        yield
        qkv_tile = self.qkv_tile
        rs = buf.rs
        for i in range(DEPTH):
            b = f"{pre}blocks.{i}."
            rs_q = rs if i > 0 else None
            ops.gemm(buf.h, P[b + "attn.qkv.fold.w"], buf.qkv, M=M, N=3 * D, K=D, bias=P[b + "attn.qkv.fold.b"],
                     ln_in=(None if rs_q is not None else buf.part, P[b + "attn.qkv.fold.s"]), ln_rs_in=rs_q,
                     tile=qkv_tile)
            if "attn" not in _ABLATE:
                ops.attention(buf.qkv, buf.a, n_img, TOK, HEADS, D // HEADS, log2q=True)
            ops.gemm(buf.a, P[b + "attn.proj.weight"], None, M=M, N=D, K=D,
                     bias=P[b + "attn.proj.bias"], gamma=P[b + "ls1.gamma"], accumulate=True,
                     ln_out=(buf.h, buf.part), ln_xl=buf.xl, ln_rs_out=rs)
            ops.gemm(buf.h, P[b + "mlp.fc1.fold.w"], buf.m, M=M, N=MLP_DIM, K=D, bias=P[b + "mlp.fc1.fold.b"],
                     act=DP_ACT_GELU, ln_in=(None, P[b + "mlp.fc1.fold.s"]), ln_rs_in=rs)
            last = i == DEPTH - 1
            need_x = last or bool(hooks and i in hooks)
            ops.gemm(buf.m, P[b + "mlp.fc2.weight"], buf.x if need_x else None, M=M, N=D, K=MLP_DIM,
                     bias=P[b + "mlp.fc2.bias"], gamma=P[b + "ls2.gamma"], accumulate=True,
                     ln_out=(buf.h, None if last else buf.part), ln_xl=buf.xl, ln_rs_out=None if last else rs)
            if hooks and i in hooks:
                hooks[i]()
            if last:
                ops.layernorm(buf.x, P[pre + "norm.weight"], P[pre + "norm.bias"], buf.out, M, D)
            yield

    def _conv3(self, x, s_in, cin, w, out, cout, bias=None, relu_a=False, act=0, R1=None, R2=None,
               stride=1, border_corr=None, tile=0):
        s_out = (s_in + 2 - 3) // stride + 1
        ops.gemm(x, w, out, M=s_out * s_out, N=cout, K=9 * cin,
                 conv=dict(in_h=s_in, in_w=s_in, in_c=cin, k=3, stride=stride, pad=1, out_h=s_out, out_w=s_out),
                 relu_a=relu_a, bias=bias, act=act, R1=R1, ldr1=cout, R2=R2, ldr2=cout, ldc=cout,
                 border_corr=border_corr, tile=tile)

    def _deconv(self, x, s_in, cin, w, out, cout, bias=None, C_off=0, ldc=None):
        ops.gemm(x, w, out, M=s_in * s_in, N=4 * cout, K=cin, bias=bias, deconv=(s_in, s_in, cout),
                 C_off=C_off, ldc=cout if ldc is None else ldc)

    def _resblock(self, pre: str, x, s, out, extra=None, t=None):
        P = self.P
        if t is None:
            t = self.dec[s]["t"]
            self._resblock_head(pre, x, s, t)
        self._conv3(t, s, 256, P[pre + ".3.w"], out, 256, bias=P[pre + ".3.b"], R1=x, R2=extra)

    def _resblock_head(self, pre: str, x, s, t):
        P = self.P
        self._conv3(x, s, 256, P[pre + ".1.w"], t, 256, bias=P[pre + ".1.b"], relu_a=True, act=DP_ACT_RELU)

    def _fusion(self, i: int, feats, s, x1, t1=None):
        P, d = self.P, self.dec[s]
        p = f"decoder.fusions.{i}."
        x = feats
        if x1 is not None:
            self._resblock(p + "resnet1", x1, s, d["x"], extra=feats, t=t1)
            x = d["x"]
        self._resblock(p + "resnet2", x, s, d["y"])
        if i != 0:
            out = self.up[2 * s]
            self._deconv(d["y"], s, 256, P[p + "up.w"], out, 256, bias=P[p + "up.b"])
            return out
        if self.head0_compose:
            return d["y"]
        ops.gemm(d["y"], P[p + "out.w"], self.feats, M=s * s, N=256, K=256, bias=P[p + "out.b"])
        return self.feats

    def _side_encoders(self):
        for _ in self._side_steps():
            pass

    def _side_steps(self):
        P, e = self.P, "encoder."
        yield from self._vit_steps(self.side_vits, self.vs, 1, 34 * PTOK)
        ops.merge_windows(self.vi.out, 0, 1, 0, self.g)
        self._deconv(self.g, 24, D, P[e + "upsample_lowres.w"], self.cat, D, bias=P[e + "upsample_lowres.b"],
                     C_off=D, ldc=2 * D)
        if self.use_fov:
            ops.gemm(self.vf.out, P["fov.lin.w"], self.fov_tok, M=PTOK, N=128, K=D, A_off=D, bias=P["fov.lin.b"])

    def _fov_head(self):
        P = self.P
        self._conv3(self.low, 48, 256, P["fov.down.w"], self.fx, 128, bias=P["fov.down.b"], act=DP_ACT_RELU,
                    R1=self.fov_tok, stride=2)
        self._conv3(self.fx, 24, 128, P["fov.h0.w"], self.f12, 64, bias=P["fov.h0.b"], act=DP_ACT_RELU, stride=2)
        self._conv3(self.f12, 12, 64, P["fov.h2.w"], self.f6, 32, bias=P["fov.h2.b"], act=DP_ACT_RELU, stride=2)
        ops.fov_tail(self.f6, P["fov.h4.w"], P["fov.h4.b"], self.fov_deg)

    def forward(self) -> Tuple[torch.Tensor, torch.Tensor]:
        with ops.use_workspace(self.ws_main):
            out = self._forward()
        for i, w in enumerate(self._wss):
            ops.workspace_check(w, self.status_dev[i:i + 1])
        return out

    def _on(self, st: torch.cuda.Stream, after=None):
        main = torch.cuda.current_stream(self.dev)
        if self.serial_side:
            return ops.use_workspace(self.ws_main)
        if isinstance(after, torch.cuda.Event):
            st.wait_event(after)
        else:
            st.wait_stream(after if after is not None else main)
        return _StreamCtx(st)

    def _forward(self) -> Tuple[torch.Tensor, torch.Tensor]:
        P, e = self.P, "encoder."
        main = torch.cuda.current_stream(self.dev)
        serial = self.serial_side
        side_ok = "side" not in _ABLATE

        def mark(st):
            ev = torch.cuda.Event()
            ev.record(main if serial else st)
            return ev

        ops.patchify_pyramid(self.x0, self.cols)
        if side_ok:
            with self._on(self.side):
                self._side_encoders()
        vp = self.vp
        ev = {}

        def lat0_chain():
            with self._on(self.dec_a):
                ops.gemm(self.lat0, P[e + "upsample_latent0.0"], self.t96_256, M=96 * 96, N=256, K=D)
                self._deconv(self.t96_256, 96, 256, P[e + "upsample_latent0.1"], self.t192_256, 256)
                self._deconv(self.t192_256, 192, 256, P[e + "upsample_latent0.2"], self.t384_256, 256)
                ev["lat0pre"] = mark(self.dec_a)

        def lat1_chain():
            with self._on(self.dec_b):
                ops.gemm(self.lat1, P[e + "upsample_latent1.0"], self.t96_256b, M=96 * 96, N=256, K=D)
                self._deconv(self.t96_256b, 96, 256, P[e + "upsample_latent1.1"], self.t192_256b, 256)
                self._deconv(self.t192_256b, 192, 256, P[e + "upsample_latent1.2"], self.enc1, 256)
                ev["enc1"] = mark(self.dec_b)

        hooks = {5: lambda: ops.merge_windows(vp.x, 0, 5, 3, self.lat0),
                 11: lambda: ops.merge_windows(vp.x, 0, 5, 3, self.lat1)}
        self._vit(["encoder.patch_encoder."], vp, NWIN, 0, hooks)
        ops.merge_windows(vp.out, 0, 5, 3, self.f0)
        ops.merge_windows(vp.out, 25, 3, 6, self.f1)
        ops.merge_windows(vp.out, 34, 1, 0, self.f2)

        early = "decoder" not in _ABLATE
        t1 = self.dec[768]["c"] if early else None
        lat0_chain()
        with self._on(self.dec_b):
            ops.gemm(self.f1, P[e + "upsample1.0"], self.t48_1024, M=48 * 48, N=D, K=D)
            self._deconv(self.t48_1024, 48, D, P[e + "upsample1.1"], self.enc3, D)
            ev["enc3"] = mark(self.dec_b)
            ops.gemm(self.f0, P[e + "upsample0.0"], self.t96_512, M=96 * 96, N=512, K=D)
            self._deconv(self.t96_512, 96, 512, P[e + "upsample0.1"], self.enc2, 512)
            ev["enc2"] = mark(self.dec_b)
        lat1_chain()
        sk = DP_TILE_SPLITK_256x256
        ops.gemm(self.f2, P[e + "upsample2.0"], self.t24_1024, M=24 * 24, N=D, K=D)
        self._deconv(self.t24_1024, 24, D, P[e + "upsample2.1"], self.cat, D, ldc=2 * D)
        if not serial:
            main.wait_stream(self.side)
        ops.gemm(self.cat, P[e + "fuse_lowres.w"], self.enc4, M=48 * 48, N=D, K=2 * D, bias=P[e + "fuse_lowres.b"])
        self._conv3(self.enc4, 48, D, P["decoder.convs.4"], self.low, 256,
                    tile=sk)
        with self._on(self.dec_c), ops.use_workspace(self.ws_main if serial else self.ws_dec):
            for i, (enc, s_, cin) in ((3, (self.enc3, 96, D)), (2, (self.enc2, 192, 512)),
                                      (1, (self.enc1, 384, 256))):
                if not serial:
                    self.dec_c.wait_event(ev[f"enc{i}"])
                self._conv3(enc, s_, cin, P[f"decoder.convs.{i}"], self.dec[s_]["c"], 256)
                ev[f"c{i}"] = mark(self.dec_c)
            if not serial:
                self.dec_c.wait_event(ev["lat0pre"])
            self._deconv(self.t384_256, 384, 256, P[e + "upsample_latent0.3"], self.enc0, 256)
            ev["enc0"] = mark(self.dec_c)
            if early:
                self._resblock_head("decoder.fusions.0.resnet1", self.enc0, 768, t1)
                ev["r1a"] = mark(self.dec_c)
            if self.use_fov and side_ok:
                if not serial:
                    self.dec_c.wait_stream(self.side)
                self._fov_head()
        if "decoder" not in _ABLATE:
            f = self._fusion(4, self.low, 48, None)
            for i, s in ((3, 96), (2, 192), (1, 384)):
                if not serial:
                    main.wait_event(ev[f"c{i}"])
                    if i == 1:
                        main.wait_event(ev["enc0"])
                f = self._fusion(i, f, s, self.dec[s]["c"])
            if early and not serial:
                main.wait_event(ev["r1a"])
            feats = self._fusion(0, f, 768, self.enc0, t1=t1)
        else:
            feats = self.feats
        if not serial:
            for st in (self.dec_a, self.dec_b, self.dec_c, self.side):
                main.wait_stream(st)
        if "head" in _ABLATE:
            return self.canonical, self.fov_deg
        if self.head0_compose and "decoder" not in _ABLATE:
            self._conv3(feats, 768, 256, P["head.0c.w"], self.h0, 128, bias=P["head.0c.b"],
                        border_corr=P["head.0c.corr"])
        else:
            self._conv3(feats, 768, 256, P["head.0.w"], self.h0, 128, bias=P["head.0.b"])
        taps = 4 if self.head_ps_compact else 9
        ops.gemm(self.h0, P["head.ps.w4" if self.head_ps_compact else "head.ps.w"], self.canonical,
                 M=768 * 768, N=128, K=taps * 128,
                 conv=dict(in_h=768, in_w=768, in_c=128, k=3, stride=1, pad=1, out_h=768, out_w=768),
                 bias=P["head.ps.b"], head_w=P["head.4.w"], head_b=P["head.4.b"], head_corr=P["head.ps.corr"])
        return self.canonical, self.fov_deg

    def capture_graph(self) -> None:
        s = torch.cuda.Stream(device=self.dev)
        s.wait_stream(torch.cuda.current_stream(self.dev))
        with torch.cuda.stream(s):
            self.forward()
        torch.cuda.current_stream(self.dev).wait_stream(s)
        g = torch.cuda.CUDAGraph()
        with torch.cuda.graph(g):
            self.forward()
        self.graph = g

    def run(self) -> Tuple[torch.Tensor, torch.Tensor]:
        if self.graph is not None:
            self.graph.replay()
        else:
            self.forward()
        return self.canonical, self.fov_deg

    def finish_status(self) -> FrameStatus:
        words = torch.empty(self.status_dev.numel(), dtype=torch.int32, pin_memory=True)
        words.copy_(self.status_dev, non_blocking=True)
        self.status_dev[-1:].zero_()
        ev = torch.cuda.Event()
        ev.record()
        st = FrameStatus(self._frames, words, ev)
        self._frames += 1
        self._recent.append(st)
        if len(self._recent) > 64:
            self._sweep(block_oldest=True)
        self.last_status = st
        if self.sync_check:
            st.check()
        return st

    def _sweep(self, block: bool = False, block_oldest: bool = False) -> None:
        keep = []
        for j, st in enumerate(self._recent):
            if st.reported or st.owned:
                continue
            if block or st.ready() or (block_oldest and j == 0):
                if st.error() is not None:
                    self._unreported.append(st)
            else:
                keep.append(st)
        self._recent = keep

    def check_status(self, block: bool = True) -> None:
        self._sweep(block=block)
        bad, self._unreported = [st for st in self._unreported if not (st.reported or st.owned)], []
        if bad:
            for st in bad:
                st.reported = True
            raise DPError("; ".join(f"frame {st.frame}: {st.error()}" for st in bad))


class _StreamCtx:

    def __init__(self, st):
        self.st = torch.cuda.stream(st)
        self.ws = ops.use_workspace(None)

    def __enter__(self):
        self.st.__enter__()
        self.ws.__enter__()
        return self

    def __exit__(self, *exc):
        self.ws.__exit__(*exc)
        return self.st.__exit__(*exc)
```

ml-depth-pro-video_amd/depth_pro/ops.py:

```python

from __future__ import annotations

import ctypes
from typing import Optional

import torch

from . import _lib
from ._lib import (DP_A_CONV, DP_A_DENSE, DP_ACT_NONE, DP_BF16, DP_F16, DP_F32,
                   DP_STORE_DECONV2X2, DP_STORE_HEAD_PS, DP_STORE_ROWS, GemmArgs, check)

_TORCH_DT = {DP_BF16: torch.bfloat16, DP_F16: torch.float16, DP_F32: torch.float32}


def torch_dtype(code: int) -> torch.dtype:
    return _TORCH_DT[code]


def dtype_code(dt: torch.dtype) -> int:
    for k, v in _TORCH_DT.items():
        if v == dt:
            return k
    raise _lib.DPError(f"unsupported dtype {dt}")


_PROF: Optional[list] = None
_PROF_T0: Optional[torch.cuda.Event] = None
PROF_GEMM_META: dict = {}


def profile_begin() -> None:
    global _PROF, _PROF_T0
    _PROF = []
    _PROF_T0 = torch.cuda.Event(enable_timing=True)
    _PROF_T0.record()


def profile_end(timeline: bool = False) -> list:
    global _PROF
    rec, _PROF = _PROF or [], None
    torch.cuda.synchronize()
    if timeline:
        return [(k, f, sh, dt, _PROF_T0.elapsed_time(a), _PROF_T0.elapsed_time(b), st)
                for (k, f, sh, dt, a, b, st) in rec]
    return [(k, f, sh, dt, a.elapsed_time(b)) for (k, f, sh, dt, a, b, st) in rec]


class _Timed:
    def __init__(self, kind: str, flops: float, shape: tuple = (), dtype=None):
        self.kind, self.flops, self.shape, self.dtype = kind, flops, shape, dtype

    def __enter__(self):
        if _PROF is not None:
            self.e0 = torch.cuda.Event(enable_timing=True)
            self.e1 = torch.cuda.Event(enable_timing=True)
            self.e0.record()
        return self

    def __exit__(self, *exc):
        if _PROF is not None:
            self.e1.record()
            _PROF.append((self.kind, self.flops, self.shape, self.dtype, self.e0, self.e1,
                          torch.cuda.current_stream().cuda_stream))
        return False


_WS: Optional[torch.Tensor] = None


class use_workspace:

    def __init__(self, ws: Optional[torch.Tensor]):
        self.ws = ws

    def __enter__(self):
        global _WS
        self.prev, _WS = _WS, self.ws
        return self

    def __exit__(self, *exc):
        global _WS
        _WS = self.prev
        return False


WS_ERROR_OFFSET = 4092


def workspace_error(ws: torch.Tensor) -> int:
    return int(ws[WS_ERROR_OFFSET:WS_ERROR_OFFSET + 4].view(torch.int32).item())


def workspace_check(ws: torch.Tensor, status: torch.Tensor) -> None:
    check(_lib.load().dp_gemm_workspace_check(ws.data_ptr(), status.data_ptr(), _stream(status)),
          "dp_gemm_workspace_check")


def gemm_workspace(device: torch.device) -> torch.Tensor:
    return torch.zeros(int(_lib.load().dp_gemm_workspace_size()), dtype=torch.uint8, device=device)


def conv_weight(w: torch.Tensor, dt: Optional[torch.dtype] = None) -> torch.Tensor:
    co, ci, kh, kw = w.shape
    if ci % 64:
        raise _lib.DPError(f"conv input channels must be a multiple of 64, got {ci}")
    b = w.reshape(co, ci // 64, 64, kh, kw).permute(0, 1, 3, 4, 2).reshape(co, -1)
    return (b if dt is None else b.to(dt)).contiguous()


def _stream(t: torch.Tensor) -> int:
    return torch.cuda.current_stream(t.device).cuda_stream


def _p(t: Optional[torch.Tensor]) -> Optional[int]:
    return None if t is None else t.data_ptr()


def gemm(A: torch.Tensor, B: torch.Tensor, C: torch.Tensor, *, M: int, N: int, K: int,
         lda: Optional[int] = None, ldb: Optional[int] = None, ldc: Optional[int] = None,
         conv: Optional[dict] = None, relu_a: bool = False,
         bias: Optional[torch.Tensor] = None, act: int = DP_ACT_NONE,
         gamma: Optional[torch.Tensor] = None,
         pos: Optional[torch.Tensor] = None, ldpos: int = 0, pos_group: int = 0, pos_off: int = 0,
         R1: Optional[torch.Tensor] = None, ldr1: int = 0,
         R2: Optional[torch.Tensor] = None, ldr2: int = 0,
         accumulate: bool = False, deconv: Optional[tuple] = None,
         row_group: int = 0, row_group_out: int = 0, row_off: int = 0,
         head_w: Optional[torch.Tensor] = None, head_b: float = 0.0,
         head_corr: Optional[torch.Tensor] = None,
         A_off: int = 0, C_off: int = 0, B_off: int = 0, tile: int = 0,
         workspace: Optional[torch.Tensor] = None,
         plan_only: bool = False, border_corr: Optional[torch.Tensor] = None,
         ln_out: Optional[tuple] = None, ln_in: Optional[tuple] = None, ln_eps: float = 1e-6,
         ln_xl: Optional[torch.Tensor] = None, ln_rs_out: Optional[torch.Tensor] = None,
         ln_rs_in: Optional[torch.Tensor] = None):
    if C is None:
        if ln_xl is None:
            raise _lib.DPError("dp_gemm: C is required (only a split-residual producer may omit it)")
        C = torch.empty(0, dtype=torch.float32, device=ln_xl.device)
    a = _gemm_args(A, B, C, M=M, N=N, K=K, lda=lda, ldb=ldb, ldc=ldc, conv=conv, relu_a=relu_a, bias=bias,
                   act=act, gamma=gamma, pos=pos, ldpos=ldpos, pos_group=pos_group, pos_off=pos_off, R1=R1,
                   ldr1=ldr1, R2=R2, ldr2=ldr2, accumulate=accumulate, deconv=deconv, row_group=row_group,
                   row_group_out=row_group_out, row_off=row_off, head_w=head_w, head_b=head_b,
                   head_corr=head_corr, A_off=A_off, C_off=C_off, B_off=B_off, tile=tile, workspace=workspace,
                   border_corr=border_corr)
    if ln_out is not None:
        xb, part = ln_out
        if xb.numel() < (M - 1) * a.ldc + N or xb.dtype != B.dtype or (part is None and ln_xl is None) or \
                (part is not None and (part.numel() < M * (N // 128) * 2 or part.dtype != torch.float32)):
            raise _lib.DPError("dp_gemm: ln_out buffers too small or of the wrong type")
        a.ln_xb_out, a.ln_part_out = xb.data_ptr(), _p(part)
    if ln_xl is not None:
        if ln_out is None or ln_xl.numel() < (M - 1) * a.ldc + N or ln_xl.dtype != torch.int8:
            raise _lib.DPError("dp_gemm: ln_xl needs ln_out and [M][ldc] int8 rows")
        a.ln_xl = ln_xl.data_ptr()
        if C.numel() == 0:
            a.C = None
    if ln_rs_out is not None:
        if ln_out is None or ln_rs_out.numel() < 2 * M or ln_rs_out.dtype != torch.float32:
            raise _lib.DPError("dp_gemm: ln_rs_out needs ln_out and fp32 [M][2]")
        a.ln_rs_out, a.ln_eps = ln_rs_out.data_ptr(), float(ln_eps)
    if ln_in is not None:
        part, colsum = ln_in
        if (part is None) == (ln_rs_in is None) or colsum.numel() < N or colsum.dtype != torch.float32 or \
                (part is not None and part.numel() < M * (K // 128) * 2) or \
                (ln_rs_in is not None and (ln_rs_in.numel() < 2 * (M + (M & 1)) or ln_rs_in.dtype != torch.float32)):
            raise _lib.DPError("dp_gemm: ln_in buffers too small or of the wrong type")
        a.ln_part_in, a.ln_colsum, a.ln_eps = _p(part), colsum.data_ptr(), float(ln_eps)
        a.ln_rs_in = _p(ln_rs_in)
    elif ln_rs_in is not None:
        raise _lib.DPError("dp_gemm: ln_rs_in needs ln_in=(None, colsum)")
    if plan_only:
        t, g = ctypes.c_int32(), ctypes.c_int32()
        check(_lib.load().dp_gemm_plan(ctypes.byref(a), ctypes.byref(t), ctypes.byref(g)), "dp_gemm_plan")
        return t.value, g.value
    _check_gemm_extents(A, B, C if a.C else None, a, A_off, C_off, conv, deconv, head_w is not None,
                        head_corr is not None, B_off)
    kind = "gemm_conv" if conv is not None else ("gemm_deconv" if deconv is not None else "gemm")
    if _PROF is not None:
        PROF_GEMM_META[(kind, (M, N, K), B.dtype)] = {"act": int(act), "ln_consumer": bool(a.ln_colsum),
                                                     "deconv": deconv is not None}
    with _Timed(kind, 2.0 * M * N * K, (M, N, K), B.dtype):
        check(_lib.load().dp_gemm(ctypes.byref(a), _stream(B)), "dp_gemm")


def gemm_grouped(groups, **common) -> None:
    arr = (GemmArgs * len(groups))()
    for i, g in enumerate(groups):
        kw = dict(common)
        kw.update(g)
        A, B, C = kw.pop("A"), kw.pop("B"), kw.pop("C")
        arr[i] = _gemm_args(A, B, C, **kw)
        _check_gemm_extents(A, B, C, arr[i], kw.get("A_off", 0), kw.get("C_off", 0), None, None, False, False)
    M, N, K = common["M"], common["N"], common["K"]
    with _Timed("gemm", 2.0 * M * N * K * len(groups), (M, N, K), groups[0]["B"].dtype):
        check(_lib.load().dp_gemm_grouped(arr, len(groups), _stream(groups[0]["C"])), "dp_gemm_grouped")


def _gemm_args(A, B, C, *, M, N, K, lda=None, ldb=None, ldc=None, conv=None, relu_a=False, bias=None,
               act=DP_ACT_NONE, gamma=None, pos=None, ldpos=0, pos_group=0, pos_off=0, R1=None, ldr1=0, R2=None,
               ldr2=0, accumulate=False, deconv=None, row_group=0, row_group_out=0, row_off=0, head_w=None,
               head_b=0.0, head_corr=None, A_off=0, C_off=0, B_off=0, tile=0, workspace=None,
               border_corr=None) -> "GemmArgs":
    a = GemmArgs()
    a.M, a.N, a.K = M, N, K
    a.dtype = dtype_code(B.dtype)
    a.A = A.data_ptr() + A_off * A.element_size()
    a.lda = K if lda is None else lda
    a.B = B.data_ptr() + B_off * B.element_size()
    a.ldb = K if ldb is None else ldb
    if conv is not None:
        a.a_mode = DP_A_CONV
        a.in_h, a.in_w, a.in_c = conv["in_h"], conv["in_w"], conv["in_c"]
        a.k_h, a.k_w = conv["k"], conv["k"]
        a.stride, a.pad = conv.get("stride", 1), conv.get("pad", 0)
        a.out_h, a.out_w = conv["out_h"], conv["out_w"]
        a.lda = 0
    else:
        a.a_mode = DP_A_DENSE
    a.relu_a = int(relu_a)
    a.bias = _p(bias)
    a.act = act
    a.gamma = _p(gamma)
    a.pos = _p(pos)
    a.ldpos, a.pos_group, a.pos_off = ldpos, pos_group, pos_off
    a.R1, a.ldr1 = _p(R1), ldr1
    a.R2, a.ldr2 = _p(R2), ldr2
    a.C = C.data_ptr() + C_off * C.element_size()
    a.ldc = N if ldc is None else ldc
    a.c_dtype = dtype_code(C.dtype)
    a.accumulate = int(accumulate)
    if deconv is not None:
        a.store_mode = DP_STORE_DECONV2X2
        a.dc_h, a.dc_w, a.dc_cout = deconv
    elif head_corr is not None:
        a.store_mode = DP_STORE_HEAD_PS
    else:
        a.store_mode = DP_STORE_ROWS
    a.row_group, a.row_group_out, a.row_off = row_group, row_group_out, row_off
    a.head_w = _p(head_w)
    a.head_b = float(head_b)
    if border_corr is not None and border_corr.numel() < 9 * N:
        raise _lib.DPError("dp_gemm: border_corr needs 9 * N values")
    a.head_corr = _p(head_corr if head_corr is not None else border_corr)
    a.tile = tile
    ws = workspace if workspace is not None else _WS
    if ws is not None:
        a.workspace, a.workspace_bytes = ws.data_ptr(), ws.numel() * ws.element_size()
    return a


def _check_gemm_extents(A, B, C, a, A_off, C_off, conv, deconv, head, head_ps, B_off=0) -> None:
    def need(t, off, n, what):
        if off + n > t.numel():
            raise _lib.DPError(f"dp_gemm: {what} needs {off + n} elements, tensor has {t.numel()}")

    M, N, K = a.M, a.N, a.K
    if conv is not None:
        need(A, A_off, (M // (a.out_h * a.out_w)) * a.in_h * a.in_w * a.in_c, "A (conv input)")
    else:
        need(A, A_off, (M - 1) * a.lda + K, "A")
    need(B, B_off, (N - 1) * a.ldb + K, "B")
    if C is None:
        return
    if head_ps:
        need(C, C_off, (M // (a.out_h * a.out_w)) * 4 * a.out_h * a.out_w, "C (pixel-shuffle head)")
    elif head:
        need(C, C_off, M, "C (fused head)")
    elif deconv is not None:
        need(C, C_off, (4 * M - 1) * a.ldc + a.dc_cout, "C (deconv)")
    else:
        last = M - 1
        if a.row_group:
            last = (last // a.row_group) * a.row_group_out + a.row_off + last % a.row_group
        need(C, C_off, last * a.ldc + N, "C")


def layernorm(x: torch.Tensor, w: torch.Tensor, b: torch.Tensor, y: torch.Tensor, rows: int, cols: int,
              eps: float = 1e-6) -> None:
    with _Timed("layernorm", 0.0, (rows, cols), y.dtype):
        check(_lib.load().dp_layernorm(x.data_ptr(), cols, w.data_ptr(), b.data_ptr(), y.data_ptr(), cols,
                                       rows, cols, eps, dtype_code(y.dtype), _stream(y)), "dp_layernorm")


def layernorm_stats(x: torch.Tensor, xb: torch.Tensor, part: torch.Tensor, rows: int, cols: int,
                    xl: Optional[torch.Tensor] = None) -> None:
    if x.numel() < rows * cols or xb.numel() < rows * cols or part.numel() < rows * (cols // 128) * 2:
        raise _lib.DPError("dp_layernorm_stats: buffers smaller than rows * cols")
    if xl is not None and (xl.numel() < rows * cols or xl.dtype != torch.int8):
        raise _lib.DPError("dp_layernorm_stats: xl must be int8 rows * cols")
    with _Timed("layernorm", 0.0, (rows, cols), xb.dtype):
        check(_lib.load().dp_layernorm_stats(x.data_ptr(), cols, rows, cols, xb.data_ptr(), cols,
                                             xl.data_ptr() if xl is not None else None, part.data_ptr(),
                                             dtype_code(xb.dtype), _stream(xb)), "dp_layernorm_stats")


def split_residual(x: torch.Tensor, dt: torch.dtype):
    s = 16 if dt == torch.bfloat16 else 19
    hi = x.to(dt)
    hf = hi.float()
    e = torch.frexp(hf).exponent
    q = torch.round(torch.ldexp(x.float() - hf, (s - e).float())).clamp(-128, 127).to(torch.int8)
    return hi, q


def merge_residual(hi: torch.Tensor, q: torch.Tensor) -> torch.Tensor:
    s = 16 if hi.dtype == torch.bfloat16 else 19
    hf = hi.float()
    e = torch.frexp(hf).exponent
    return hf + torch.ldexp(q.float(), (e - s).float())


def fold_layernorm(w: torch.Tensor, b: torch.Tensor, ln_w: torch.Tensor, ln_b: torch.Tensor, dt: torch.dtype,
                   col_scale: Optional[torch.Tensor] = None):
    w64, b64 = w.double(), b.double()
    s = torch.ones(w.shape[0], dtype=torch.float64, device=w.device) if col_scale is None else col_scale.double()
    wf = (w64 * ln_w.double()[None, :] * s[:, None]).to(dt).contiguous()
    bias = ((b64 + w64 @ ln_b.double()) * s).float().contiguous()
    colsum = wf.double().sum(1).float().contiguous()
    return wf, bias, colsum


def layernorm_grouped(x: torch.Tensor, ws, bs, y: torch.Tensor, rows_per_group: int, cols: int,
                      eps: float = 1e-6) -> None:
    n = len(ws)
    pw = (ctypes.c_void_p * n)(*[t.data_ptr() for t in ws])
    pb = (ctypes.c_void_p * n)(*[t.data_ptr() for t in bs])
    if x.numel() < n * rows_per_group * cols or y.numel() < n * rows_per_group * cols:
        raise _lib.DPError("dp_layernorm_grouped: x / y smaller than groups * rows_per_group * cols")
    with _Timed("layernorm", 0.0, (n * rows_per_group, cols), y.dtype):
        check(_lib.load().dp_layernorm_grouped(x.data_ptr(), cols, pw, pb, n, y.data_ptr(), cols, rows_per_group,
                                               cols, eps, dtype_code(y.dtype), _stream(y)), "dp_layernorm_grouped")


def attention(qkv: torch.Tensor, out: torch.Tensor, batch: int, seq: int, heads: int = 16,
              head_dim: int = 64, log2q: bool = False, scale: Optional[float] = None) -> None:
    if log2q and scale is not None:
        raise _lib.DPError("dp_attention_log2q takes no scale: it is folded into Q")
    with _Timed("attention", 4.0 * batch * heads * seq * seq * head_dim, (batch, seq), out.dtype):
        if log2q:
            check(_lib.load().dp_attention_log2q(qkv.data_ptr(), out.data_ptr(), batch, seq, heads, head_dim,
                                                 dtype_code(out.dtype), _stream(out)), "dp_attention_log2q")
        else:
            check(_lib.load().dp_attention(qkv.data_ptr(), out.data_ptr(), batch, seq, heads, head_dim,
                                           head_dim ** -0.5 if scale is None else float(scale),
                                           dtype_code(out.dtype), _stream(out)), "dp_attention")


LOG2E = 1.4426950408889634


def log2q_gamma(heads: int, head_dim: int, device) -> torch.Tensor:
    g = torch.ones(3 * heads * head_dim, dtype=torch.float32)
    g[:heads * head_dim] = float(head_dim ** -0.5 * LOG2E)
    return g.to(device)


def normalize_u8(img: torch.Tensor, out: torch.Tensor) -> None:
    H, W = img.shape[0], img.shape[1]
    check(_lib.load().dp_normalize_u8(img.data_ptr(), H, W, out.data_ptr(), dtype_code(out.dtype),
                                      _stream(out)), "dp_normalize_u8")


def interp_mode(mode: str) -> int:
    if mode not in _lib.INTERP_MODES:
        raise ValueError(f"interpolation_mode={mode!r}: expected one of {sorted(_lib.INTERP_MODES)}")
    return _lib.INTERP_MODES[mode]


def resize(src: torch.Tensor, dst: torch.Tensor, mode: str = "bilinear") -> None:
    src = src.contiguous()
    C, H, W = src.shape[-3:]
    OH, OW = dst.shape[-2:]
    check(_lib.load().dp_resize(src.data_ptr(), dtype_code(src.dtype), C, H, W, dst.data_ptr(),
                                OH, OW, interp_mode(mode), _stream(dst)), "dp_resize")


def resize_bilinear(src: torch.Tensor, dst: torch.Tensor) -> None:
    resize(src, dst, "bilinear")


def patchify_pyramid(x0: torch.Tensor, cols: torch.Tensor) -> None:
    check(_lib.load().dp_patchify_pyramid(x0.data_ptr(), cols.data_ptr(), dtype_code(cols.dtype),
                                          _stream(cols)), "dp_patchify_pyramid")


def vit_cls_rows(x: torch.Tensor, cls: torch.Tensor, pos: torch.Tensor, n: int) -> None:
    check(_lib.load().dp_vit_cls_rows(x.data_ptr(), cls.data_ptr(), pos.data_ptr(), n, _stream(x)),
          "dp_vit_cls_rows")


def merge_windows(src: torch.Tensor, first_window: int, steps: int, padding: int, dst: torch.Tensor,
                  ld: int = 1024, windows: Optional[tuple] = None) -> None:
    lib = _lib.load()
    if windows is None:
        check(lib.dp_merge_windows(src.data_ptr(), dtype_code(src.dtype), ld, first_window, steps, padding,
                                   dst.data_ptr(), dtype_code(dst.dtype), _stream(dst)), "dp_merge_windows")
    else:
        check(lib.dp_merge_windows_range(src.data_ptr(), dtype_code(src.dtype), ld, first_window, steps, padding,
                                         int(windows[0]), int(windows[1]), dst.data_ptr(), dtype_code(dst.dtype),
                                         _stream(dst)), "dp_merge_windows_range")


def fov_tail(x6: torch.Tensor, w: torch.Tensor, bias: float, out: torch.Tensor) -> None:
    check(_lib.load().dp_fov_tail(x6.data_ptr(), dtype_code(x6.dtype), w.data_ptr(), float(bias),
                                  out.data_ptr(), _stream(out)), "dp_fov_tail")


def infer_epilogue(canonical: torch.Tensor, fov_deg: Optional[torch.Tensor], f_given: Optional[float],
                   H: int, W: int, depth: torch.Tensor, f_px_out: Optional[torch.Tensor],
                   nonfinite: Optional[torch.Tensor] = None, mode: str = "bilinear") -> None:
    SH, SW = canonical.shape[-2:]
    use_given = f_given is not None
    check(_lib.load().dp_infer_epilogue_mode(canonical.data_ptr(), SH, SW, _p(fov_deg), int(use_given),
                                             float(f_given) if use_given else 0.0, H, W, depth.data_ptr(),
                                             _p(f_px_out), _p(nonfinite), interp_mode(mode), _stream(depth)),
          "dp_infer_epilogue_mode")


def resize_u8_cv(img: torch.Tensor, out_h: int, out_w: int, area: bool) -> torch.Tensor:
    if img.dtype != torch.uint8 or img.dim() != 3 or img.shape[2] != 3:
        raise _lib.DPError(f"resize_u8_cv expects a uint8 HxWx3 tensor, got {img.dtype} {tuple(img.shape)}")
    img = img.contiguous()
    H, W = img.shape[0], img.shape[1]
    out = torch.empty(out_h, out_w, 3, dtype=torch.uint8, device=img.device)
    interp = _lib.DP_CV_INTER_AREA if area else _lib.DP_CV_INTER_LINEAR
    check(_lib.load().dp_resize_u8_cv(img.data_ptr(), H, W, out.data_ptr(), out_h, out_w, interp, _stream(out)),
          "dp_resize_u8_cv")
    return out


_LUTS = {}


def colormap_lut(cmap: str, device: torch.device):
    key = (cmap, str(device))
    if key not in _LUTS:
        import matplotlib.pyplot as plt
        import numpy as np

        m = plt.get_cmap(cmap)
        n = m.N
        rgba = np.concatenate([m(np.arange(n)), m(np.array([-1.0])), m(np.array([2.0])), m(np.array([np.nan]))])
        lut = (rgba[:, :3] * 255).astype(np.uint8)
        _LUTS[key] = (torch.from_numpy(lut).to(device), n)
    return _LUTS[key]


def depth_to_image(depth: torch.Tensor, colored: bool = True, cmap: str = "turbo",
                   out: Optional[torch.Tensor] = None, scratch: Optional[torch.Tensor] = None) -> torch.Tensor:
    if depth.dtype != torch.float32 or not depth.is_contiguous():
        raise _lib.DPError("depth_to_image expects a contiguous fp32 depth map")
    H, W = depth.shape[-2:]
    if scratch is None:
        scratch = torch.empty(2, dtype=torch.int32, device=depth.device)
    if colored:
        lut, n = colormap_lut(cmap, depth.device)
        if out is None:
            out = torch.empty(H, W, 3, dtype=torch.uint8, device=depth.device)
        mode, lp = _lib.DP_DEPTH_IMG_COLOR, lut.data_ptr()
    else:
        if out is None:
            out = torch.empty(H, W, dtype=torch.int16, device=depth.device)
        mode, lp, n = _lib.DP_DEPTH_IMG_RAW16, None, 0
    check(_lib.load().dp_depth_to_image(depth.data_ptr(), H * W, scratch.data_ptr(), lp, n, mode, out.data_ptr(),
                                        _stream(depth)), "dp_depth_to_image")
    return out
```

Measured before the change: 53.97 frames/sec.

## Fold LayerNorm into grouped side-ViT GEMMs via partial stats epilogues

```diff
diff --git a/ml-depth-pro-video_amd/csrc/dp_gemm.hip b/ml-depth-pro-video_amd/csrc/dp_gemm.hip
--- a/ml-depth-pro-video_amd/csrc/dp_gemm.hip
+++ b/ml-depth-pro-video_amd/csrc/dp_gemm.hip
@@ -360,9 +360,22 @@
   for (int g = 0; g < groups; ++g) {
     GemmP q;
     int t = 0;
-    const int rc = gemm_plan(&a[g], q, t);
+    dp_gemm_args plain = a[g];
+    plain.ln_part_out = nullptr; plain.ln_xb_out = nullptr; plain.ln_part_in = nullptr; plain.ln_colsum = nullptr;
+    const dp_gemm_args &x = a[0], &y = a[g];
+    const bool lnp = y.ln_part_out || y.ln_xb_out, lnc = y.ln_part_in || y.ln_colsum;
+    const int rc = gemm_plan(&plain, q, t);
     if (rc) return rc;
-    const dp_gemm_args &x = a[0], &y = a[g];
+    if (lnp && (lnc || !y.ln_part_out || !y.ln_xb_out || !y.accumulate || y.c_dtype != DP_F32 || y.act != DP_ACT_NONE ||
+                y.N % 128 != 0 || y.R1 || y.R2 || y.pos || y.row_group))
+      return DP_ERR_ARG;
+    if (lnc && (!y.ln_part_in || !y.ln_colsum || y.K != 1024 || y.accumulate || y.c_dtype == DP_F32 || y.gamma ||
+                (y.act != DP_ACT_NONE && y.act != DP_ACT_GELU) || !(y.ln_eps > 0.f) || y.ldc % 8 != 0 || y.R1 || y.R2 ||
+                y.pos || y.row_group))
+      return DP_ERR_ARG;
+    if (!y.ln_part_out != !x.ln_part_out || !y.ln_xb_out != !x.ln_xb_out || !y.ln_part_in != !x.ln_part_in ||
+        !y.ln_colsum != !x.ln_colsum || ((lnc) && y.ln_eps != x.ln_eps))
+      return DP_ERR_ARG;
     if (y.M != x.M || y.N != x.N || y.K != x.K || y.dtype != x.dtype || y.lda != x.lda || y.ldb != x.ldb ||
         y.a_mode != DP_A_DENSE || x.a_mode != DP_A_DENSE || y.relu_a || y.act != x.act ||
         !y.bias != !x.bias || !y.gamma != !x.gamma || !y.pos != !x.pos || y.ldpos != x.ldpos ||
@@ -370,12 +383,14 @@
         !y.R2 != !x.R2 || y.ldr2 != x.ldr2 || y.ldc != x.ldc || y.c_dtype != x.c_dtype ||
         y.accumulate != x.accumulate || y.store_mode != DP_STORE_ROWS || x.store_mode != DP_STORE_ROWS ||
         y.row_group != x.row_group || y.row_group_out != x.row_group_out || y.row_off != x.row_off ||
-        y.head_w || y.head_corr || y.N % 8 != 0 || y.ln_part_out || y.ln_xb_out || y.ln_xl || y.ln_part_in ||
-        y.ln_rs_out || y.ln_rs_in ||
-        y.ln_colsum)
-      return DP_ERR_ARG;
-    if (g == 0) p = q;
-    p.grp[g] = GemmP::Group{q.A, q.B, q.bias, q.gamma, q.pos, q.R1, q.R2, q.C};
+        y.head_w || y.head_corr || y.N % 8 != 0 || y.ln_xl || y.ln_rs_out || y.ln_rs_in)
+      return DP_ERR_ARG;
+    if (g == 0) {
+      p = q;
+      p.ln_eps = y.ln_eps;
+    }
+    p.grp[g] = GemmP::Group{q.A, q.B, q.bias, q.gamma, q.pos, q.R1, q.R2, q.C,
+                            y.ln_part_out, (u16*)y.ln_xb_out, y.ln_part_in, y.ln_colsum};
   }
   p.groups = groups;
   hipStream_t s = (hipStream_t)stream;
diff --git a/ml-depth-pro-video_amd/csrc/dp_gemm_big.h b/ml-depth-pro-video_amd/csrc/dp_gemm_big.h
--- a/ml-depth-pro-video_amd/csrc/dp_gemm_big.h
+++ b/ml-depth-pro-video_amd/csrc/dp_gemm_big.h
@@ -2,6 +2,7 @@
 
 #include "dp_gemm_dev.h"
 #include "dp_gemm_epilogue.h"
+#include "dp_ln_merge.h"
 
 namespace {
 
@@ -42,6 +43,8 @@
     const GemmP::Group& q = p_arg.grp[g];
     p_grp.A = q.A; p_grp.B = q.B; p_grp.bias = q.bias; p_grp.gamma = q.gamma; p_grp.pos = q.pos;
     p_grp.R1 = q.R1; p_grp.R2 = q.R2; p_grp.C = q.C;
+    p_grp.ln_part_out = q.ln_part_out; p_grp.ln_xb_out = q.ln_xb_out;
+    p_grp.ln_part_in = q.ln_part_in; p_grp.ln_colsum = q.ln_colsum;
   }
   int kbeg = 0, kcnt = p_arg.K / BKT;
   if constexpr (SPLIT) {
@@ -63,6 +66,16 @@
   const int m0 = tile_m * BM, n0 = tile_n * BN;
   DP_STAMPS_DECL;
   DP_STAMP(st0_);
+  constexpr bool LNP = EACT == EPI_LNP, LNC = EACT >= EPI_LNC;
+  static_assert(!(LNP || LNC) || (GRP && BM == 128 && BN == 128 && NW == 8), "folded LN: the grouped 128 x 128 tile");
+  f32x4_t lnc_part[4];
+  if constexpr (LNC) {
+    if (tid < BM) {
+      const f32x4_t* pp = (const f32x4_t*)(p.ln_part_in + (long long)min(m0 + tid, p.M - 1) * 16);
+      #pragma unroll
+      for (int i = 0; i < 4; ++i) lnc_part[i] = pp[i];
+    }
+  }
 
   const int prow = wave * ROWS_PER_WAVE_PIECE + lane / CR;
   const int pchunk = BKT == 64 ? ((lane & 7) ^ ((lane >> 3) & 7)) : ((lane & 3) ^ ((lane >> 3) & 3));
@@ -252,7 +265,27 @@
       for (int j = 0; j < FN; ++j) asm volatile("" ::"v"(acc[i][j][0]), "v"(acc[i][j][1]), "v"(acc[i][j][2]), "v"(acc[i][j][3]));
     return;
   }
-  if constexpr (EACT >= EPI_ACC) {
+  if constexpr (LNC) {
+    __shared__ float2 ln_rs_s[BM];
+    if (tid < BM) ln_rs_s[tid] = ln_merge_row(lnc_part, p.ln_eps);
+    lds_barrier();
+    constexpr int PF = (FM * 16 * TN * 2 * NW <= SMEM) ? FM : FM / 2;
+    epilogue_mfma<K_, EACT - EPI_LNC, FM, FN, TN, PF, true>(p, acc, smem + wave * (PF * 16 * TN * 2), lane,
+                                                             m0 + wm * TM, n0 + wn * TN, ln_rs_s + wm * TM);
+    return;
+  } else if constexpr (LNP) {
+    static_assert(WN == 4 && TN == 32, "one 128-column chunk over 4 waves");
+    __shared__ f32x4_t ln_st[BM * 4];
+    epilogue_acc32_ln<K_, FM, FN>(p, acc, ln_st + wm * TM * 4 + wn, lane, m0 + wm * TM, n0 + wn * TN);
+    lds_barrier();
+    if (tid < BM && m0 + tid < p.M) {
+      f32x4_t e[4];
+      #pragma unroll
+      for (int w = 0; w < 4; ++w) e[w] = ln_st[tid * 4 + w];
+      *(float2*)(p.ln_part_out + ((long long)(m0 + tid) * (p.N / 128) + n0 / 128) * 2) = ln_chunk_merge(e);
+    }
+    return;
+  } else if constexpr (EACT >= EPI_ACC) {
     epilogue_acc32<EACT - EPI_ACC, FM, FN>(p, acc, lane, m0 + wm * TM, n0 + wn * TN);
     return;
   } else if constexpr (EACT >= 0) {
@@ -318,7 +351,16 @@
       if (conv || p.relu_a) return DP_ERR_ARG;
       dim3 g(p.tiles_n * p.tiles_m * p.groups);
 #define DP_GRP(E_) hipLaunchKernelGGL((gemm_big_kernel<K_, BM, BN, 64, 3, true, false, false, 8, E_, true>), g, dim3(NT_BIG), 0, s, p)
-      if (ea == DP_ACT_NONE) DP_GRP(DP_ACT_NONE);
+      const bool lnp = p.grp[0].ln_part_out, lnc = p.grp[0].ln_part_in;
+      if constexpr (BM == 128) {
+        if (lnp) DP_GRP(EPI_LNP);
+        else if (lnc && p.act == DP_ACT_GELU) DP_GRP(EPI_LNC + DP_ACT_GELU);
+        else if (lnc) DP_GRP(EPI_LNC + DP_ACT_NONE);
+      } else if (lnp || lnc) {
+        return DP_ERR_ARG;
+      }
+      if (lnp || lnc) {  }
+      else if (ea == DP_ACT_NONE) DP_GRP(DP_ACT_NONE);
       else if (ea == DP_ACT_GELU) DP_GRP(DP_ACT_GELU);
       else if (ea == EPI_ACC) DP_GRP(EPI_ACC);
       else DP_GRP(-1);
diff --git a/ml-depth-pro-video_amd/csrc/dp_gemm_epilogue.h b/ml-depth-pro-video_amd/csrc/dp_gemm_epilogue.h
--- a/ml-depth-pro-video_amd/csrc/dp_gemm_epilogue.h
+++ b/ml-depth-pro-video_amd/csrc/dp_gemm_epilogue.h
@@ -147,12 +147,69 @@
   }
 }
 
-template <typename K_, int ACT, int FM, int FN, int TN, int PF>
+template <typename K_, int ACT, int FM, int FN, int TN, int PF, bool LNC = false>
 __device__ __forceinline__ void epilogue_mfma(const GemmP& p, f32x4_t (&acc)[FM][FN], char* slab, int lane,
-                                              int m_base, int n_base) {
+                                              int m_base, int n_base, const float2* rsm = nullptr) {
   constexpr int CH = TN / 8;
   constexpr int RPI = 64 / CH;
   static_assert(FM % PF == 0 && (CH == 16 || CH == 8 || CH == 4), "tile");
+  const int t = lane & 15, g = lane >> 4;
+  float bias[FN][4], gam[FN][4];
+  #pragma unroll
+  for (int fn = 0; fn < FN; ++fn) {
+    const int n = n_base + fn * 16 + 4 * g;
+    const bool ok = n < p.N;
+    const float4 b = (p.bias && ok) ? *(const float4*)(p.bias + n) : make_float4(0.f, 0.f, 0.f, 0.f);
+    float4 q;
+    if constexpr (LNC) q = ok ? *(const float4*)(p.ln_colsum + n) : make_float4(0.f, 0.f, 0.f, 0.f);
+    else q = (p.gamma && ok) ? *(const float4*)(p.gamma + n) : make_float4(1.f, 1.f, 1.f, 1.f);
+    bias[fn][0] = b.x; bias[fn][1] = b.y; bias[fn][2] = b.z; bias[fn][3] = b.w;
+    gam[fn][0] = q.x; gam[fn][1] = q.y; gam[fn][2] = q.z; gam[fn][3] = q.w;
+  }
+  #pragma unroll
+  for (int f0 = 0; f0 < FM; f0 += PF) {
+    #pragma unroll
+    for (int fm = 0; fm < PF; ++fm)
+      #pragma unroll
+      for (int fn = 0; fn < FN; ++fn) {
+        f32x4_t x;
+        if constexpr (LNC) {
+          const float2 rs = rsm[(f0 + fm) * 16 + t];
+          x = __builtin_elementwise_fma(
+              acc[f0 + fm][fn], (f32x4_t)(rs.x),
+              __builtin_elementwise_fma(f32x4_t{gam[fn][0], gam[fn][1], gam[fn][2], gam[fn][3]}, (f32x4_t)(rs.y),
+                                        f32x4_t{bias[fn][0], bias[fn][1], bias[fn][2], bias[fn][3]}));
+        } else {
+          x = acc[f0 + fm][fn] + f32x4_t{bias[fn][0], bias[fn][1], bias[fn][2], bias[fn][3]};
+        }
+        if constexpr (ACT == DP_ACT_RELU) {
+          #pragma unroll
+          for (int r = 0; r < 4; ++r) x[r] = fmaxf(x[r], 0.f);
+        } else if constexpr (ACT == DP_ACT_GELU) {
+          x = gelu_erf4(x);
+        }
+        if constexpr (!LNC) x = x * f32x4_t{gam[fn][0], gam[fn][1], gam[fn][2], gam[fn][3]};
+        const int row = fm * 16 + t;
+        const int chunk = fn * 2 + (g >> 1);
+        uint2 w;
+        w.x = K_::pack2(x[0], x[1]);
+        w.y = K_::pack2(x[2], x[3]);
+        *(uint2*)(slab + row * (TN * 2) + ((chunk ^ (row & (CH - 1))) << 4) + (g & 1) * 8) = w;
+      }
+    #pragma unroll
+    for (int k = 0; k < PF * 16 / RPI; ++k) {
+      const int row = k * RPI + lane / CH, chunk = lane % CH;
+      const uint4 d = *(const uint4*)(slab + row * (TN * 2) + ((chunk ^ (row & (CH - 1))) << 4));
+      const int m = m_base + f0 * 16 + row, n = n_base + chunk * 8;
+      if (m < p.M && n < p.N) *(uint4*)((u16*)p.C + (long long)m * p.ldc + n) = d;
+    }
+  }
+}
+
+template <int ACT, int FM, int FN>
+__device__ __forceinline__ void epilogue_acc32(const GemmP& p, f32x4_t (&acc)[FM][FN], int lane, int m_base,
+                                               int n_base) {
+  #pragma clang fp contract(off)
   const int t = lane & 15, g = lane >> 4;
   float bias[FN][4], gam[FN][4];
   #pragma unroll
@@ -164,52 +221,6 @@
     bias[fn][0] = b.x; bias[fn][1] = b.y; bias[fn][2] = b.z; bias[fn][3] = b.w;
     gam[fn][0] = q.x; gam[fn][1] = q.y; gam[fn][2] = q.z; gam[fn][3] = q.w;
   }
-  #pragma unroll
-  for (int f0 = 0; f0 < FM; f0 += PF) {
-    #pragma unroll
-    for (int fm = 0; fm < PF; ++fm)
-      #pragma unroll
-      for (int fn = 0; fn < FN; ++fn) {
-        f32x4_t x = acc[f0 + fm][fn] + f32x4_t{bias[fn][0], bias[fn][1], bias[fn][2], bias[fn][3]};
-        if constexpr (ACT == DP_ACT_RELU) {
-          #pragma unroll
-          for (int r = 0; r < 4; ++r) x[r] = fmaxf(x[r], 0.f);
-        } else if constexpr (ACT == DP_ACT_GELU) {
-          x = gelu_erf4(x);
-        }
-        x = x * f32x4_t{gam[fn][0], gam[fn][1], gam[fn][2], gam[fn][3]};
-        const int row = fm * 16 + t;
-        const int chunk = fn * 2 + (g >> 1);
-        uint2 w;
-        w.x = K_::pack2(x[0], x[1]);
-        w.y = K_::pack2(x[2], x[3]);
-        *(uint2*)(slab + row * (TN * 2) + ((chunk ^ (row & (CH - 1))) << 4) + (g & 1) * 8) = w;
-      }
-    #pragma unroll
-    for (int k = 0; k < PF * 16 / RPI; ++k) {
-      const int row = k * RPI + lane / CH, chunk = lane % CH;
-      const uint4 d = *(const uint4*)(slab + row * (TN * 2) + ((chunk ^ (row & (CH - 1))) << 4));
-      const int m = m_base + f0 * 16 + row, n = n_base + chunk * 8;
-      if (m < p.M && n < p.N) *(uint4*)((u16*)p.C + (long long)m * p.ldc + n) = d;
-    }
-  }
-}
-
-template <int ACT, int FM, int FN>
-__device__ __forceinline__ void epilogue_acc32(const GemmP& p, f32x4_t (&acc)[FM][FN], int lane, int m_base,
-                                               int n_base) {
-  #pragma clang fp contract(off)
-  const int t = lane & 15, g = lane >> 4;
-  float bias[FN][4], gam[FN][4];
-  #pragma unroll
-  for (int fn = 0; fn < FN; ++fn) {
-    const int n = n_base + fn * 16 + 4 * g;
-    const bool ok = n < p.N;
-    const float4 b = (p.bias && ok) ? *(const float4*)(p.bias + n) : make_float4(0.f, 0.f, 0.f, 0.f);
-    const float4 q = (p.gamma && ok) ? *(const float4*)(p.gamma + n) : make_float4(1.f, 1.f, 1.f, 1.f);
-    bias[fn][0] = b.x; bias[fn][1] = b.y; bias[fn][2] = b.z; bias[fn][3] = b.w;
-    gam[fn][0] = q.x; gam[fn][1] = q.y; gam[fn][2] = q.z; gam[fn][3] = q.w;
-  }
   float* const C = (float*)p.C;
   f32x4_t cur[FN], nxt[FN];
   auto load_row = [&](int fm, f32x4_t (&c)[FN]) __attribute__((always_inline)) {
@@ -234,6 +245,76 @@
       }
       if (m < p.M) *(f32x4_t*)(C + (long long)m * p.ldc + n_base + fn * 16 + 4 * g) = x;
     }
+    #pragma unroll
+    for (int fn = 0; fn < FN; ++fn) cur[fn] = nxt[fn];
+  }
+}
+
+template <typename K_, int FM, int FN>
+__device__ __forceinline__ void epilogue_acc32_ln(const GemmP& p, f32x4_t (&acc)[FM][FN], f32x4_t* st, int lane,
+                                                  int m_base, int n_base) {
+  #pragma clang fp contract(off)
+  const int t = lane & 15, g = lane >> 4;
+  float bias[FN][4], gam[FN][4];
+  #pragma unroll
+  for (int fn = 0; fn < FN; ++fn) {
+    const int n = n_base + fn * 16 + 4 * g;
+    const float4 b = p.bias ? *(const float4*)(p.bias + n) : make_float4(0.f, 0.f, 0.f, 0.f);
+    const float4 q = p.gamma ? *(const float4*)(p.gamma + n) : make_float4(1.f, 1.f, 1.f, 1.f);
+    bias[fn][0] = b.x; bias[fn][1] = b.y; bias[fn][2] = b.z; bias[fn][3] = b.w;
+    gam[fn][0] = q.x; gam[fn][1] = q.y; gam[fn][2] = q.z; gam[fn][3] = q.w;
+  }
+  float* const C = (float*)p.C;
+  f32x4_t cur[FN], nxt[FN];
+  auto load_row = [&](int fm, f32x4_t (&c)[FN]) __attribute__((always_inline)) {
+    const int m = min(m_base + fm * 16 + t, p.M - 1);
+    #pragma unroll
+    for (int fn = 0; fn < FN; ++fn) c[fn] = *(const f32x4_t*)(C + (long long)m * p.ldc + n_base + fn * 16 + 4 * g);
+  };
+  load_row(0, cur);
+  #pragma unroll
+  for (int fm = 0; fm < FM; ++fm) {
+    if (fm + 1 < FM) load_row(fm + 1, nxt);
+    const int m = m_base + fm * 16 + t;
+    f32x4_t x[FN];
+    #pragma unroll
+    for (int fn = 0; fn < FN; ++fn) {
+      #pragma unroll
+      for (int r = 0; r < 4; ++r) {
+        const float v = acc[fm][fn][r] + bias[fn][r];
+        x[fn][r] = v * gam[fn][r] + cur[fn][r];
+      }
+      if (m < p.M) {
+        *(f32x4_t*)(C + (long long)m * p.ldc + n_base + fn * 16 + 4 * g) = x[fn];
+        uint2 w;
+        w.x = K_::pack2(x[fn][0], x[fn][1]);
+        w.y = K_::pack2(x[fn][2], x[fn][3]);
+        *(uint2*)(p.ln_xb_out + (long long)m * p.ldc + n_base + fn * 16 + 4 * g) = w;
+      }
+    }
+    const float sh = __shfl(x[0][0], t);
+    float d[FN][4], s1 = 0.f;
+    #pragma unroll
+    for (int fn = 0; fn < FN; ++fn)
+      #pragma unroll
+      for (int r = 0; r < 4; ++r) {
+        d[fn][r] = x[fn][r] - sh;
+        s1 += d[fn][r];
+      }
+    s1 += __shfl_xor(s1, 16);
+    s1 += __shfl_xor(s1, 32);
+    const float dm = s1 * (1.f / 32);
+    float s2 = 0.f;
+    #pragma unroll
+    for (int fn = 0; fn < FN; ++fn)
+      #pragma unroll
+      for (int r = 0; r < 4; ++r) {
+        const float e = d[fn][r] - dm;
+        s2 += e * e;
+      }
+    s2 += __shfl_xor(s2, 16);
+    s2 += __shfl_xor(s2, 32);
+    if (g == 0) st[(fm * 16 + t) * 4] = f32x4_t{sh, dm, s2, 0.f};
     #pragma unroll
     for (int fn = 0; fn < FN; ++fn) cur[fn] = nxt[fn];
   }
diff --git a/ml-depth-pro-video_amd/csrc/dp_gemm_impl.h b/ml-depth-pro-video_amd/csrc/dp_gemm_impl.h
--- a/ml-depth-pro-video_amd/csrc/dp_gemm_impl.h
+++ b/ml-depth-pro-video_amd/csrc/dp_gemm_impl.h
@@ -64,6 +64,10 @@
     const u16* R1;
     const u16* R2;
     void* C;
+    float* ln_part_out;
+    u16* ln_xb_out;
+    const float* ln_part_in;
+    const float* ln_colsum;
   } grp[DP_MAX_GROUPS];
 };
 
@@ -172,6 +176,7 @@
 }
 
 constexpr int EPI_ACC = 16;
+constexpr int EPI_LNP = 32, EPI_LNC = 48;
 __host__ inline int fast_epi_act(const GemmP& p) {
   if (p.dbg & DBG_NO_FAST_EPILOGUE) return -1;
   if (!needs_rowld(p)) return p.c_dtype == DP_F32 ? -1 : p.act;
diff --git a/ml-depth-pro-video_amd/csrc/dp_ln_merge.h b/ml-depth-pro-video_amd/csrc/dp_ln_merge.h
--- a/ml-depth-pro-video_amd/csrc/dp_ln_merge.h
+++ b/ml-depth-pro-video_amd/csrc/dp_ln_merge.h
@@ -17,4 +17,19 @@
   return make_float2(rs, -rs * mean);
 }
 
+__device__ __forceinline__ float2 ln_chunk_merge(const f32x4_t (&e)[4]) {
+  #pragma clang fp contract(off)
+  float mu[4];
+  #pragma unroll
+  for (int w = 0; w < 4; ++w) mu[w] = (e[w][0] - e[0][0]) + e[w][1];
+  const float mr = ((mu[0] + mu[1]) + (mu[2] + mu[3])) * 0.25f;
+  float m2 = 0.f;
+  #pragma unroll
+  for (int w = 0; w < 4; ++w) {
+    const float dl = mu[w] - mr;
+    m2 += e[w][2] + 32.f * dl * dl;
+  }
+  return make_float2(e[0][0] + mr, m2);
 }
+
+}
diff --git a/ml-depth-pro-video_amd/depth_pro/engine.py b/ml-depth-pro-video_amd/depth_pro/engine.py
--- a/ml-depth-pro-video_amd/depth_pro/engine.py
+++ b/ml-depth-pro-video_amd/depth_pro/engine.py
@@ -16,6 +16,10 @@
 
 def ln_fold_enabled() -> bool:
     return not ({"ln", "vitgemm"} & _ABLATE)
+
+
+def side_ln_fold_enabled() -> bool:
+    return ln_fold_enabled() and "sideln" not in _ABLATE
 
 
 NWIN = 35
@@ -89,40 +93,49 @@
     return v, d
 
 
+def pack_vit(sd: Dict[str, torch.Tensor], vit: str, device: torch.device, vdt, blocks=None) -> Dict[str, object]:
+    g = lambda k: sd[k].detach().to(device)
+    P: Dict[str, object] = {}
+    side = vit != "encoder.patch_encoder."
+    folded = side_ln_fold_enabled() if side else ln_fold_enabled()
+    blocks = range(DEPTH) if blocks is None else blocks
+    P[vit + "cls"] = _f32(g(vit + "cls_token")).reshape(D)
+    P[vit + "pos"] = _f32(g(vit + "pos_embed")).reshape(TOK, D)
+    P[vit + "pe.w"] = g(vit + "patch_embed.proj.weight").reshape(D, -1).to(vdt).contiguous()
+    P[vit + "pe.b"] = _f32(g(vit + "patch_embed.proj.bias"))
+    for i in blocks:
+        b = f"{vit}blocks.{i}."
+        for n in ("norm1.weight", "norm1.bias", "norm2.weight", "norm2.bias", "attn.qkv.bias",
+                  "attn.proj.bias", "mlp.fc1.bias", "mlp.fc2.bias", "ls1.gamma", "ls2.gamma"):
+            if folded and side and n.startswith("norm"):
+                continue
+            P[b + n] = _f32(g(b + n))
+        for n in ("attn.qkv.weight", "attn.proj.weight", "mlp.fc1.weight", "mlp.fc2.weight"):
+            if folded and n in ("attn.qkv.weight", "mlp.fc1.weight"):
+                continue
+            P[b + n] = g(b + n).to(vdt).contiguous()
+    P[vit + "norm.weight"] = _f32(g(vit + "norm.weight"))
+    P[vit + "norm.bias"] = _f32(g(vit + "norm.bias"))
+    if folded:
+        qg = ops.log2q_gamma(HEADS, D // HEADS, device)
+        for i in blocks:
+            b = f"{vit}blocks.{i}."
+            for lin, ln, cs in (("attn.qkv", "norm1", qg), ("mlp.fc1", "norm2", None)):
+                wf, bf, sf = ops.fold_layernorm(g(b + lin + ".weight").float(), g(b + lin + ".bias").float(),
+                                                g(b + ln + ".weight").float(), g(b + ln + ".bias").float(),
+                                                vdt, cs)
+                P[b + lin + ".fold.w"], P[b + lin + ".fold.b"], P[b + lin + ".fold.s"] = wf, bf, sf
+    return P
+
+
 def pack_weights(sd: Dict[str, torch.Tensor], device: torch.device, dtype_code) -> Dict[str, object]:
     vcode, dcode = precision_codes(dtype_code)
     vdt, dt = ops.torch_dtype(vcode), ops.torch_dtype(dcode)
     g = lambda k: sd[k].detach().to(device)
     P: Dict[str, object] = {}
-    fold = ln_fold_enabled()
     for vit in ("encoder.patch_encoder.", "encoder.image_encoder.", "fov.encoder.0."):
-        if vit + "cls_token" not in sd:
-            continue
-        folded = fold and vit == "encoder.patch_encoder."
-        P[vit + "cls"] = _f32(g(vit + "cls_token")).reshape(D)
-        P[vit + "pos"] = _f32(g(vit + "pos_embed")).reshape(TOK, D)
-        P[vit + "pe.w"] = g(vit + "patch_embed.proj.weight").reshape(D, -1).to(vdt).contiguous()
-        P[vit + "pe.b"] = _f32(g(vit + "patch_embed.proj.bias"))
-        for i in range(DEPTH):
-            b = f"{vit}blocks.{i}."
-            for n in ("norm1.weight", "norm1.bias", "norm2.weight", "norm2.bias", "attn.qkv.bias",
-                      "attn.proj.bias", "mlp.fc1.bias", "mlp.fc2.bias", "ls1.gamma", "ls2.gamma"):
-                P[b + n] = _f32(g(b + n))
-            for n in ("attn.qkv.weight", "attn.proj.weight", "mlp.fc1.weight", "mlp.fc2.weight"):
-                if folded and n in ("attn.qkv.weight", "mlp.fc1.weight"):
-                    continue
-                P[b + n] = g(b + n).to(vdt).contiguous()
-        P[vit + "norm.weight"] = _f32(g(vit + "norm.weight"))
-        P[vit + "norm.bias"] = _f32(g(vit + "norm.bias"))
-        if folded:
-            qg = ops.log2q_gamma(HEADS, D // HEADS, device)
-            for i in range(DEPTH):
-                b = f"{vit}blocks.{i}."
-                for lin, ln, cs in (("attn.qkv", "norm1", qg), ("mlp.fc1", "norm2", None)):
-                    wf, bf, sf = ops.fold_layernorm(g(b + lin + ".weight").float(), g(b + lin + ".bias").float(),
-                                                    g(b + ln + ".weight").float(), g(b + ln + ".bias").float(),
-                                                    vdt, cs)
-                    P[b + lin + ".fold.w"], P[b + lin + ".fold.b"], P[b + lin + ".fold.s"] = wf, bf, sf
+        if vit + "cls_token" in sd:
+            P.update(pack_vit(sd, vit, device, vdt))
     for name, n_up in (("upsample_latent0", 3), ("upsample_latent1", 2), ("upsample0", 1),
                        ("upsample1", 1), ("upsample2", 1)):
         p = f"encoder.{name}."
@@ -175,10 +188,10 @@
 
 
 class _ViTBuffers:
-    def __init__(self, rows: int, dt, dev, out_dt=None, ln_fold: bool = False):
+    def __init__(self, rows: int, dt, dev, out_dt=None, ln_fold: bool = False, part: bool = False):
         self.rows = rows
         self.x = torch.empty(rows, D, dtype=torch.float32, device=dev)
-        self.part = torch.empty(rows, D // 128, 2, dtype=torch.float32, device=dev) if ln_fold else None
+        self.part = torch.empty(rows, D // 128, 2, dtype=torch.float32, device=dev) if ln_fold or part else None
         self.h = torch.empty(rows, D, dtype=dt, device=dev)
         self.xl = torch.empty(rows, D, dtype=torch.int8, device=dev) if ln_fold else None
         self.rs = (torch.empty((rows + 255) // 256 * 256, 2, dtype=torch.float32, device=dev)
@@ -273,7 +286,7 @@
         if device.index is None:
             device = torch.device("cuda", torch.cuda.current_device())
         self.vcode, self.code = precision_codes(dtype_code)
-        if packed[next(k for k in packed if k.endswith("attn.qkv.weight"))].dtype != ops.torch_dtype(self.vcode) \
+        if packed[next(k for k in packed if k.endswith("attn.proj.weight"))].dtype != ops.torch_dtype(self.vcode) \
                 or packed["decoder.convs.4"].dtype != ops.torch_dtype(self.code):
             raise DPError("packed weights were made for another compute precision")
         self.P = packed
@@ -292,7 +305,11 @@
                           "when they were packed)")
         self.vp = _ViTBuffers(NWIN * TOK, vdt, dev, dt, ln_fold=self.ln_fold)
         self.side_vits = ["encoder.image_encoder."] + (["fov.encoder.0."] if self.use_fov else [])
-        self.vs = _ViTBuffers(len(self.side_vits) * TOK, vdt, dev, dt)
+        self.side_fold = "encoder.image_encoder.blocks.0.attn.qkv.fold.w" in packed
+        if self.side_fold and not side_ln_fold_enabled():
+            raise DPError("packed weights were made for the other LayerNorm path (DP_ABLATE differs from "
+                          "when they were packed)")
+        self.vs = _ViTBuffers(len(self.side_vits) * TOK, vdt, dev, dt, part=self.side_fold)
         self.vi = _ViTRows(self.vs, 0, TOK)
         self.vf = _ViTRows(self.vs, TOK, 2 * TOK) if self.use_fov else None
         self.lat0 = e(96 * 96, D)
@@ -361,10 +378,15 @@
         def lin(A, key, C, N, K, a_rows=True, **kw):
             per = {k: kw.pop(k) for k in ("bias", "gamma", "pos") if isinstance(kw.get(k), str)}
             A_off = kw.pop("A_off", 0)
+            ln_in, ln_out = kw.pop("ln_in", None), kw.pop("ln_out", False)
             groups = []
             for g, pre in enumerate(pres):
                 d = dict(A=A, B=P[pre + key], C=C, A_off=A_off + (g * M * K if a_rows else 0), C_off=g * M * N)
                 d.update({k: P[pre + v] for k, v in per.items()})
+                if ln_in:
+                    d["ln_in"] = (buf.part[g * M:], P[pre + ln_in])
+                if ln_out:
+                    d["ln_out"] = (buf.h[g * M:], buf.part[g * M:])
                 groups.append(d)
             ops.gemm_grouped(groups, M=kw.pop("M", M), N=N, K=K, **kw)
 
@@ -377,10 +399,31 @@
             row_off=1)
         for g, pre in enumerate(pres):
             ops.vit_cls_rows(buf.x[g * M:], P[pre + "cls"], P[pre + "pos"], n_img)
-        if G == 1 and buf.part is not None:
+        if G == 1 and buf.xl is not None:
             yield from self._vit_blocks_folded(pres[0], buf, M, hooks)
             return
         yield
+        if buf.part is not None:
+            ops.layernorm_stats(buf.x, buf.h, buf.part, G * M, D)
+            for i in range(DEPTH):
+                b = f"blocks.{i}."
+                lin(buf.h, b + "attn.qkv.fold.w", buf.qkv, 3 * D, D, bias=b + "attn.qkv.fold.b",
+                    ln_in=b + "attn.qkv.fold.s")
+                if "attn" not in _ABLATE:
+                    ops.attention(buf.qkv, buf.a, G * n_img, TOK, HEADS, D // HEADS, log2q=True)
+                lin(buf.a, b + "attn.proj.weight", buf.x, D, D, bias=b + "attn.proj.bias", gamma=b + "ls1.gamma",
+                    accumulate=True, ln_out=True)
+                lin(buf.h, b + "mlp.fc1.fold.w", buf.m, MLP_DIM, D, bias=b + "mlp.fc1.fold.b", act=DP_ACT_GELU,
+                    ln_in=b + "mlp.fc1.fold.s")
+                last = i == DEPTH - 1
+                lin(buf.m, b + "mlp.fc2.weight", buf.x, D, MLP_DIM, bias=b + "mlp.fc2.bias", gamma=b + "ls2.gamma",
+                    accumulate=True, ln_out=not last)
+                if hooks and i in hooks:
+                    hooks[i]()
+                if last:
+                    norm("norm", buf.out)
+                yield
+            return
         for i in range(DEPTH):
             b = f"blocks.{i}."
             if ln_on:
diff --git a/ml-depth-pro-video_amd/depth_pro/ops.py b/ml-depth-pro-video_amd/depth_pro/ops.py
--- a/ml-depth-pro-video_amd/depth_pro/ops.py
+++ b/ml-depth-pro-video_amd/depth_pro/ops.py
@@ -186,13 +186,27 @@
 
 def gemm_grouped(groups, **common) -> None:
     arr = (GemmArgs * len(groups))()
+    M, N, K = common["M"], common["N"], common["K"]
     for i, g in enumerate(groups):
         kw = dict(common)
         kw.update(g)
         A, B, C = kw.pop("A"), kw.pop("B"), kw.pop("C")
+        ln_out, ln_in, ln_eps = kw.pop("ln_out", None), kw.pop("ln_in", None), kw.pop("ln_eps", 1e-6)
         arr[i] = _gemm_args(A, B, C, **kw)
-        _check_gemm_extents(A, B, C, arr[i], kw.get("A_off", 0), kw.get("C_off", 0), None, None, False, False)
-    M, N, K = common["M"], common["N"], common["K"]
+        a = arr[i]
+        _check_gemm_extents(A, B, C, a, kw.get("A_off", 0), kw.get("C_off", 0), None, None, False, False)
+        if ln_out is not None:
+            xb, part = ln_out
+            if xb.numel() < (M - 1) * a.ldc + N or xb.dtype != B.dtype or part.numel() < M * (N // 128) * 2 or \
+                    part.dtype != torch.float32:
+                raise _lib.DPError("dp_gemm_grouped: ln_out buffers too small or of the wrong type")
+            a.ln_xb_out, a.ln_part_out = xb.data_ptr(), part.data_ptr()
+        if ln_in is not None:
+            part, colsum = ln_in
+            if part.numel() < M * (K // 128) * 2 or part.dtype != torch.float32 or colsum.numel() < N or \
+                    colsum.dtype != torch.float32:
+                raise _lib.DPError("dp_gemm_grouped: ln_in buffers too small or of the wrong type")
+            a.ln_part_in, a.ln_colsum, a.ln_eps = part.data_ptr(), colsum.data_ptr(), float(ln_eps)
     with _Timed("gemm", 2.0 * M * N * K * len(groups), (M, N, K), groups[0]["B"].dtype):
         check(_lib.load().dp_gemm_grouped(arr, len(groups), _stream(groups[0]["C"])), "dp_gemm_grouped")
 
```

New measurement: 54.53 frames/sec, median of 6. +1.0%, better.
